# araffin/srl-zoo

Measured on AMD Instinct MI355X. Metric: images/sec (224x224x3) AE+VAE train step, higher is better.
Workload: dtype f32; 1 GPU; synthetic 224x224x3 obs, --losses autoencoder, custom_cnn, state-dim 200, bs=256 per GPU (512 frames fwd+bwd per step per GPU), Adam lr 0.005, normalised fp32 observations resident in HBM; global_batch=256, parallelism=dp1, rccl_ranks=1, devices=1

## Files before the change

### include/srlz.h

```cpp
#ifndef SRLZ_H
#define SRLZ_H

#include <stddef.h>
#include <stdint.h>

#ifdef __cplusplus
extern "C" {
#endif

typedef void* srlz_stream_t;

enum srlz_status {
  SRLZ_OK = 0,
  SRLZ_ERR_BAD_DESC = -1,
  SRLZ_ERR_WORKSPACE = -2,
  SRLZ_ERR_HIP = -3,
  SRLZ_ERR_NULL = -4
};

#define SRLZ_ABI_VERSION 104
int srlz_version(void);
const char* srlz_last_error(void);
int srlz_device_cus(void);

typedef struct {
  int n;
  int hi, wi;
  int ho, wo;
  int ksize;
  int stride;
  int pad;
  int transposed;
  int groups;
} srlz_conv64_desc;

size_t srlz_conv64_packed_floats(void);
int srlz_conv64_pack_weights(const float* w_ref, float* wpack_fwd, float* wpack_bwd,
                             const srlz_conv64_desc* d, srlz_stream_t stream);
int srlz_conv64_fwd_tiles(const srlz_conv64_desc* d);
int srlz_conv64_fwd(const float* x, const float* wpack_fwd, const float* bias, float* y, float* stats_partial,
                    const float* x_bnp, const srlz_conv64_desc* d, srlz_stream_t stream);
typedef struct {
  const float* y;
  const float* bnp;
  const float* sums;
  long long count;
  int training;
  float* dy_out;
} srlz_bn_bwd_operand;
int srlz_conv64_bwd_data(const float* dy, const float* wpack_bwd, float* dx, const srlz_bn_bwd_operand* dy_bn,
                         const srlz_conv64_desc* d, srlz_stream_t stream);
struct srlz_pool_desc_s;
int srlz_conv64_bwd_data_tiles(const srlz_conv64_desc* d);
int srlz_conv64_bwd_data_pool_sums(const float* dy, const float* wpack_bwd, float* dx, const float* pooled, const float* pool_bnp,
                                   const float* pool_y, const uint8_t* pool_argmax, const struct srlz_pool_desc_s* pd,
                                   float* bn_bwd_partial, const srlz_conv64_desc* d, srlz_stream_t stream);
int srlz_conv64_bwd_fused_supported(const srlz_conv64_desc* d);
int srlz_conv64_gather_pipe_supported(const srlz_conv64_desc* d, int backward_data);
int srlz_conv64_scatter_pipe_supported(const srlz_conv64_desc* d, int backward_data);
size_t srlz_conv64_bwd_fused_workspace(const srlz_conv64_desc* d);
int srlz_conv64_bwd_fused_bn_rows(const srlz_conv64_desc* d);
int srlz_conv64_bwd_fused_workgroups(const srlz_conv64_desc* d);
int srlz_conv64_bwd_fused(const float* x, const float* x_bnp, const float* dy, const srlz_bn_bwd_operand* dy_bn,
                          const float* wpack_bwd, float* dx, float* dw_ref, float* dbias ,
                          float* x_bn_bwd_partial , void* ws, size_t ws_bytes, const srlz_conv64_desc* d,
                          srlz_stream_t stream);
int srlz_conv64_wino_supported(const srlz_conv64_desc* d);
size_t srlz_conv64_wino_packed_floats(void);
int srlz_conv64_wino_pack_weights(const float* w_ref, float* upack_fwd, float* upack_bwd, srlz_stream_t stream);
int srlz_conv64_wino_tiles(const srlz_conv64_desc* d);
int srlz_conv64_wino_fwd(const float* x, const float* upack_fwd, const float* bias , float* y,
                         float* stats_partial , const float* x_bnp ,
                         const srlz_conv64_desc* d, srlz_stream_t stream);
int srlz_conv64_wino_bwd_data(const float* dy, const float* upack_bwd, float* dx, const srlz_conv64_desc* d, srlz_stream_t stream);
int srlz_conv64_wino_bwd_data_rows(const srlz_conv64_desc* d);
int srlz_conv64_wino_bwd_data_pool_sums(const float* dy, const float* upack_bwd, float* dx, const float* pooled, const float* pool_bnp,
                                        const float* pool_y, const uint8_t* pool_argmax, const struct srlz_pool_desc_s* pd,
                                        float* bn_bwd_partial, const srlz_conv64_desc* d, srlz_stream_t stream);
size_t srlz_conv64_wino_bwd_weight_workspace(const srlz_conv64_desc* d);
int srlz_conv64_wino_bwd_weight(const float* x, const float* dy, float* dw_ref, void* ws, size_t ws_bytes, const srlz_conv64_desc* d,
                                srlz_stream_t stream);
size_t srlz_conv64_bwd_weight_workspace(const srlz_conv64_desc* d);
int srlz_conv64_bwd_weight(const float* x, const float* dy, float* dw_ref, float* dbias, const float* x_bnp ,
                           const srlz_bn_bwd_operand* dy_bn ,
                           void* ws, size_t ws_bytes, const srlz_conv64_desc* d, srlz_stream_t stream);
int srlz_conv64_bwd_weight_plan(const srlz_conv64_desc* d, int has_x_bnp, int has_dy_bn, int out[4]);

typedef struct {
  int n, hi, wi, ho, wo;
  int cin, cout;
  int ksize, stride, pad;
  int groups;
} srlz_convn_desc;
size_t srlz_convn_packed_floats(const srlz_convn_desc* d);
int srlz_convn_pack_weights(const float* w_ref, float* wpack, const srlz_convn_desc* d, srlz_stream_t stream);
int srlz_convn_fwd_tiles(const srlz_convn_desc* d);
int srlz_convn_fwd(const float* x, const float* wpack, float* y, float* stats_partial, const float* x_bnp,
                   const srlz_convn_desc* d, srlz_stream_t stream);

typedef struct {
  int n;
  int c;
  int himg, wimg;
  int hf, wf;
  int kind;
  int groups;
} srlz_skinny_desc;

int srlz_skinny_tiles(const srlz_skinny_desc* d);
int srlz_conv1_workgroups(const srlz_skinny_desc* d);
int srlz_conv1_fwd(const float* x_nchw, const float* w_ref, float* y_nhwc, float* stats_partial,
                   const srlz_skinny_desc* d, srlz_stream_t stream);
int srlz_conv1_fwd_u8(const uint8_t* x_u8, const float* norm_lut, const float* w_ref, float* y_nhwc, float* stats_partial,
                      const srlz_skinny_desc* d, srlz_stream_t stream);
size_t srlz_skinny_bwd_weight_workspace(const srlz_skinny_desc* d);
int srlz_conv1_bwd_data(const float* dy_nhwc, const float* w_ref, float* dx_nchw, const srlz_skinny_desc* d,
                        srlz_stream_t stream);
int srlz_conv1_bwd_weight(const float* x_nchw, const float* dy_nhwc, float* dw_ref, void* ws, size_t ws_bytes,
                          const srlz_skinny_desc* d, srlz_stream_t stream);
int srlz_conv1_bwd_weight_fused(const float* x_nchw, const float* y_nhwc, const float* bnp, const uint8_t* argmax,
                                const float* dpooled, const float* sums, int training, float* dw_ref, void* ws,
                                size_t ws_bytes, const srlz_skinny_desc* d, const struct srlz_pool_desc_s* pd,
                                srlz_stream_t stream);
int srlz_conv1_bwd_weight_fused_u8(const uint8_t* x_u8, const float* norm_lut, const float* y_nhwc, const float* bnp,
                                   const uint8_t* argmax, const float* dpooled, const float* sums, int training, float* dw_ref,
                                   void* ws, size_t ws_bytes, const srlz_skinny_desc* d, const struct srlz_pool_desc_s* pd,
                                   srlz_stream_t stream);
int srlz_convT_out_fwd(const float* x_nhwc, const float* w_ref, const float* bias, float* y_nchw,
                       const float* x_bnp , const srlz_skinny_desc* d,
                       srlz_stream_t stream);
int srlz_convT_out_bwd_data(const float* dy_nchw, const float* w_ref, float* dx_nhwc, const float* x_raw,
                            const float* x_bnp, float* bn_bwd_partial, const srlz_skinny_desc* d, srlz_stream_t stream);
int srlz_convT_out_bwd_weight(const float* x_nhwc, const float* dy_nchw, float* dw_ref, float* dbias,
                              const float* x_bnp, void* ws, size_t ws_bytes, const srlz_skinny_desc* d,
                              srlz_stream_t stream);

int srlz_convT_out_bwd_fused_supported(const srlz_skinny_desc* d);
int srlz_convT_out_bwd_fused_tiles(const srlz_skinny_desc* d);
size_t srlz_convT_out_bwd_fused_workspace(const srlz_skinny_desc* d);
int srlz_convT_out_bwd_fused(const float* dy_nchw, const float* w_ref, float* dx_nhwc, const float* x_raw, const float* x_bnp,
                             float* bn_bwd_partial, float* dw_ref, float* dbias , void* ws, size_t ws_bytes,
                             const float* dy_gain_dev, float dy_gain_div, float dy_gain_coef,
                             const srlz_skinny_desc* d, srlz_stream_t stream);

int srlz_convT_out_fwd_loss_workgroups(const srlz_skinny_desc* d);
int srlz_convT_out_os_plan(const srlz_skinny_desc* d, int backward, int out[2]);
int srlz_convT_out_fwd_loss(const float* x_nhwc, const float* w_ref, const float* bias, const float* target_nchw, float* err_nchw,
                            float* dec_nchw, const float* x_bnp, double* loss_partial, const srlz_skinny_desc* d,
                            srlz_stream_t stream);
int srlz_convT_out_fwd_loss_u8(const float* x_nhwc, const float* w_ref, const float* bias, const uint8_t* target_u8,
                               const float* norm_lut, float* err_nchw, float* dec_nchw, const float* x_bnp, double* loss_partial,
                               const srlz_skinny_desc* d, srlz_stream_t stream);

int srlz_bn_finalize(const float* stats_partial, int n_partials, int groups, long long count, const float* gamma,
                     const float* beta, float eps, float momentum, int repeat, float* running_mean,
                     float* running_var, long long* num_batches_tracked ,
                     float* bnp, float* batch_stat, void* ws, size_t ws_bytes, srlz_stream_t stream);
size_t srlz_bn_finalize_chunks_workspace(int chunks, int groups);
int srlz_bn_finalize_chunks(const float* stats_partial, int tiles, int chunks, int groups, long long count, const float* gamma,
                            const float* beta, float eps, float momentum, float* running_mean, float* running_var,
                            long long* num_batches_tracked , float* bnp, void* ws, size_t ws_bytes,
                            srlz_stream_t stream);
int srlz_bn_eval_params_chunks(const float* gamma, const float* beta, const float* running_mean, const float* running_var,
                               float eps, int chunks, float* bnp, srlz_stream_t stream);
int srlz_bn_add_relu(const float* a, const float* a_bnp, const float* b, const float* b_bnp, float* out, long long pixels,
                     int chunks, int groups, srlz_stream_t stream);
int srlz_avgpool_nhwc(const float* x, float* out, int n, int hw, int c, srlz_stream_t stream);
int srlz_bn_eval_params(const float* gamma, const float* beta, const float* running_mean, const float* running_var,
                        float eps, float* bnp, srlz_stream_t stream);
int srlz_bn_replay(const float* batch_stat, float momentum, float* running_mean, float* running_var,
                   srlz_stream_t stream);
#define SRLZ_BN_REPLAY_MAX 8
typedef struct {
  const float* batch_stat;
  float* running_mean;
  float* running_var;
  long long* num_batches_tracked;
} srlz_bn_replay_item;
int srlz_bn_replay_many(const srlz_bn_replay_item* items, int n, float momentum, srlz_stream_t stream);

typedef struct srlz_pool_desc_s {
  int n, h, w;
  int hp, wp;
  int pool_pad;
  int out_nchw;
  int groups;
} srlz_pool_desc;

int srlz_bn_relu_pool_fwd(const float* y, const float* bnp, float* pooled, uint8_t* argmax,
                          const srlz_pool_desc* d, srlz_stream_t stream);
size_t srlz_bn_bwd_workspace(long long elems);
int srlz_bn_relu_pool_bwd_sums(const float* y, const float* bnp, const uint8_t* argmax, const float* dpooled,
                               const float* pooled, float* sums, float* dgamma, float* dbeta, void* ws, size_t ws_bytes,
                               const srlz_pool_desc* d, srlz_stream_t stream);
int srlz_bn_relu_pool_bwd(const float* y, const float* bnp, const uint8_t* argmax, const float* dpooled,
                          const float* pooled , float* dy, float* dgamma,
                          float* dbeta, int training, void* ws, size_t ws_bytes, const srlz_pool_desc* d,
                          srlz_stream_t stream);
int srlz_bn_relu_pool_bwd_apply(const float* y, const float* bnp, const uint8_t* argmax, const float* dpooled, const float* sums,
                                float* dy, int training, const srlz_pool_desc* d, srlz_stream_t stream);
int srlz_bn_relu_fwd(const float* y, const float* bnp, float* a, long long pixels, srlz_stream_t stream);
int srlz_bn_bwd_finalize_partials(const float* partial, int n_partials, int groups, float* sums, float* dgamma, float* dbeta,
                                  void* ws, size_t ws_bytes, srlz_stream_t stream);
int srlz_bn_relu_bwd_sums(const float* y, const float* bnp, const float* da, float* sums, float* dgamma, float* dbeta,
                          void* ws, size_t ws_bytes, long long pixels, int groups, srlz_stream_t stream);
int srlz_bn_relu_bwd(const float* y, const float* bnp, const float* da, float* dy, float* dgamma, float* dbeta,
                     int training, void* ws, size_t ws_bytes, long long pixels, int groups, srlz_stream_t stream);
int srlz_nchw_to_nhwc(const float* src, float* dst, int n, int c, int h, int w, srlz_stream_t stream);
int srlz_nhwc_to_nchw(const float* src, float* dst, int n, int c, int h, int w, srlz_stream_t stream);

int srlz_dense_supported(int M, int n, int K, int plane);
size_t srlz_dense_in_workspace(int M, int n, int K);
int srlz_dense_in_fwd(const float* x, const uint8_t* x_u8, const float* norm_lut, const float* w, const float* b, float* y, int M,
                      int n, int K, int plane, int act, void* ws, size_t ws_bytes, srlz_stream_t stream);
int srlz_dense_in_wgrad(const float* dy, const float* x, const uint8_t* x_u8, const float* norm_lut, float* dw, float* db, int M,
                        int n, int K, int plane, srlz_stream_t stream);
int srlz_dense_out_fwd(const float* z, const float* w, const float* b, float* out, int M, int n, int K, int plane,
                       srlz_stream_t stream);
int srlz_dense_out_fwd_loss_workgroups(int M, int K);
int srlz_dense_out_fwd_loss(const float* z, const float* w, const float* b, const float* target, const uint8_t* target_u8,
                            const float* norm_lut, double* partial, int M, int n, int K, int plane, int half, srlz_stream_t stream);
size_t srlz_dense_out_bwd_workspace(int M, int n, int K);
int srlz_dense_out_bwd(const float* z, const float* w, const float* b, const float* target, const uint8_t* target_u8,
                       const float* norm_lut, const float* gain, float div, float* dz, float* dw, float* db, int M, int n, int K,
                       int plane, void* ws, size_t ws_bytes, srlz_stream_t stream);
int srlz_dense_out_bwd_from(const float* dout, const float* z, const float* w, float* dz, float* dw, float* db, int M, int n, int K,
                            int plane, void* ws, size_t ws_bytes, srlz_stream_t stream);
int srlz_tanh_fwd(const float* x, float* y, int n, srlz_stream_t stream);
int srlz_tanh_bwd(const float* y, const float* dy, float* dx, int n, srlz_stream_t stream);
int srlz_add_f32(const float* a, const float* b, float* out, int n, srlz_stream_t stream);

size_t srlz_linear_workspace(int M, int N, int K);
int srlz_linear_fwd(const float* x, const float* w, const float* b, float* y, int M, int N, int K, int relu,
                    void* ws, size_t ws_bytes, srlz_stream_t stream);
int srlz_linear_fwd_res(const float* x, const float* w, const float* b, const float* res, float* y, int M, int N, int K, int relu,
                        void* ws, size_t ws_bytes, srlz_stream_t stream);
int srlz_linear_bwd_data_res(const float* dy, const float* w, const float* res, float* dx, int M, int N, int K, int Kout, void* ws,
                             size_t ws_bytes, srlz_stream_t stream);
int srlz_linear_bwd_data(const float* dy, const float* w, float* dx, int M, int N, int K, void* ws, size_t ws_bytes,
                         srlz_stream_t stream);
int srlz_linear_bwd_weight(const float* dy, const float* x, float* dw, float* db, int M, int N, int K,
                           void* ws, size_t ws_bytes, srlz_stream_t stream);
int srlz_relu_bwd_inplace(const float* y, float* dy, long long n, srlz_stream_t stream);

size_t srlz_reduce_workspace(long long n);
int srlz_sqdiff_sum(const float* a, const float* b, long long n, float* out, void* ws, size_t ws_bytes,
                    srlz_stream_t stream);
int srlz_sqdiff_sum_groups(const float* a, const float* b, long long n_per_group, int groups, float* out, void* ws,
                           size_t ws_bytes, srlz_stream_t stream);
int srlz_sqdiff_grad(const float* a, const float* b, const float* coef_dev, float coef, float* da, long long n,
                     srlz_stream_t stream);
int srlz_sqdiff_grad_groups(const float* a, const float* b, const float* coef_dev, int coef_stride, float div, float coef,
                            float* da, long long n_per_group, int groups, srlz_stream_t stream);
int srlz_pair_loss_finalize(const double* partial, int nb, long long n_per_group, int mean, float* sums, float* comb,
                            srlz_stream_t stream);
int srlz_scale_by_scalar(const float* x, const float* gain_dev, float div, float coef, float* out, long long n,
                         srlz_stream_t stream);
int srlz_sqdiff_pair_loss(const float* a, const float* b, long long n_per_group, int mean, float* sums, float* comb,
                          void* ws, size_t ws_bytes, srlz_stream_t stream);
int srlz_join2(const float* a, const float* b, float* out, long long n_each, srlz_stream_t stream);

#define SRLZ_MAX_LOSS_TERMS 15
int srlz_weighted_total(const float* const* scalars, const float* weights, int n, float* total, float* tail,
                        srlz_stream_t stream);
int srlz_weighted_total_bwd(const float* dout, const float* weights, int n, float* g, srlz_stream_t stream);
int srlz_sqdiff_mean(const float* a, const float* b, long long n, float div, float* out, void* ws, size_t ws_bytes,
                     srlz_stream_t stream);
int srlz_kl_sum(const float* mu, const float* logvar, long long n, float* out, void* ws, size_t ws_bytes,
                srlz_stream_t stream);
int srlz_kl_grad(const float* mu, const float* logvar, const float* coef_dev, float coef, float* dmu,
                 float* dlogvar, long long n, srlz_stream_t stream);
int srlz_reparam_fwd(const float* mu, const float* logvar, const float* eps, float* z, long long n,
                     srlz_stream_t stream);
int srlz_reparam_bwd(const float* dz, const float* logvar, const float* eps, float* dmu, float* dlogvar,
                     long long n, srlz_stream_t stream);
int srlz_cross_entropy(const float* logits, const int64_t* target, int B, int A, float* out, float* dlogits,
                       srlz_stream_t stream);
int srlz_prelu_fwd(const float* x, const float* slope, float* y, long long n, srlz_stream_t stream);
int srlz_prelu_bwd(const float* x, const float* slope, const float* dy, float* dx, float* dslope, long long n,
                   srlz_stream_t stream);
int srlz_triplet_fwd(const float* s, const float* p, const float* n, int B, int S, float alpha, float* out, float* hinge,
                     srlz_stream_t stream);
int srlz_triplet_bwd(const float* s, const float* p, const float* n, const float* hinge, const float* g, int B, int S,
                     float* ds, float* dp, float* dn, srlz_stream_t stream);
int srlz_cat_cols(const float* a, const float* b, float* out, int rows, int ca, int cb, srlz_stream_t stream);
int srlz_split_cols(const float* in, float* a, float* b, int rows, int ca, int cb, srlz_stream_t stream);
int srlz_sum_terms(const float* const* terms, int nterms, float* out, long long n, srlz_stream_t stream);
int srlz_concat_onehot(const float* s, const int64_t* a, float* cat, int B, int S, int A, srlz_stream_t stream);

int srlz_normalize_u8(const uint8_t* img_nhwc, float* out_ncwh, int n, int h, int w, int c, srlz_stream_t stream);
int srlz_normalize_lut(float* norm_lut, srlz_stream_t stream);
int srlz_normalize_u8_planar(const uint8_t* x_u8, const float* norm_lut, float* out, int n, int c, long long plane,
                             srlz_stream_t stream);
int srlz_copy_frames_u8(const uint8_t* src, const long long* src_index, long long src_shift, uint8_t* dst,
                        const long long* dst_index, long long dst_shift, int n, long long frame_bytes, srlz_stream_t stream);
int srlz_copy_frames_u8_strided(const uint8_t* src, const long long* src_index, long long src_shift, long long src_frame_bytes,
                                long long src_offset_bytes, uint8_t* dst, const long long* dst_index, long long dst_shift,
                                long long dst_frame_bytes, long long dst_offset_bytes, int n, long long copy_bytes, srlz_stream_t stream);
int srlz_occlude_frames_u8(const uint8_t* store, const long long* index, long long shift, const int* rects, const float* norm_lut,
                           float* out, int n, int c, int w, int h, srlz_stream_t stream);

int srlz_mask_columns(const float* x, float* y, int rows, int cols, int lo, int hi, srlz_stream_t stream);

int srlz_param_norms(const float* const* ptrs, const long long* lens, int nseg, int mode, float scale, float* norms,
                     float* out, srlz_stream_t stream);
int srlz_param_norms_grad(const float* const* ptrs, float* const* gptrs, const long long* lens, int nseg, int mode,
                          const float* norms, const float* coef_dev, float scale, srlz_stream_t stream);

int srlz_fold_grads(float* grad, float* stages, long long n, int nstage, srlz_stream_t stream);

size_t srlz_reward_prior_workspace(int S);
int srlz_reward_prior_fwd(const float* states, const float* rewards, int B, int S, float* out, double* ws, size_t ws_bytes,
                          srlz_stream_t stream);
int srlz_reward_prior_bwd(const float* states, const float* rewards, const double* ws, size_t ws_bytes, const float* g, int B, int S,
                          float* dstates, srlz_stream_t stream);
size_t srlz_episode_prior_workspace(int B, int S);
int srlz_episode_prior_fwd(const float* states, const int* others, const float* same, int B, int S, const float* w1, const float* b1,
                           const float* w2, const float* b2, const float* w3, const float* b3, float* out, void* ws, size_t ws_bytes,
                           unsigned* ticket, srlz_stream_t stream);
int srlz_episode_prior_bwd(const float* states, const int* others, const float* same, const float* g, int B, int S, const float* w1,
                           const float* w2, const float* w3, void* ws, size_t ws_bytes, float* dstates, float* dw1, float* db1,
                           float* dw2, float* db2, float* dw3, float* db3, srlz_stream_t stream);

int srlz_adam_step(float* p, const float* g, float* m, float* v, long long n, double lr, double beta1, double beta2,
                   double eps, int step, float grad_scale, srlz_stream_t stream);
int srlz_adam_step_dev(float* p, const float* g, float* m, float* v, long long n, double lr, double beta1, double beta2,
                       double eps, int* step_dev, float* bc_dev, float grad_scale, srlz_stream_t stream);

size_t srlz_comm_unique_id_bytes(void);
int srlz_comm_unique_id(void* id_out_host);
int srlz_comm_init(const void* id_host, int rank, int world);
int srlz_comm_world(void);
int srlz_comm_allreduce_f32(float* buf, long long n, srlz_stream_t stream);
int srlz_comm_destroy(void);

int srlz_mse_target_fwd(const float* pred, const float* target, int B, int S, float* loss, float* dpred_unit, srlz_stream_t stream);
int srlz_dropout_fwd(const float* x, const unsigned char* mask, float keep, float* y, int rows, int cols, srlz_stream_t stream);
int srlz_dropout_bwd(const float* dy, const unsigned char* mask, float keep, float* dx, int rows, int cols, srlz_stream_t stream);

size_t srlz_knn_workspace(int N, int Q, int D, int K);
int srlz_knn_f64(const double* db , int N, const double* queries , int Q, int D, int K, int* idx ,
                 double* dist2 , void* ws, size_t ws_bytes, srlz_stream_t stream);

size_t srlz_gtc_workspace(int N, int G, int S);
int srlz_gtc_rows_f64(const double* gt , const double* states , int N, int G, int S, double* corr ,
                      double* colstats , void* ws, size_t ws_bytes, srlz_stream_t stream);

int srlz_reward_probe_chunk_rows(int S);
int srlz_reward_probe_fit(const float* states , const int* labels , int N, int S, const int* idx ,
                          const int* idx_host , int n_steps, int B, float* params, float* m, float* v, int t0, double lr,
                          double beta1, double beta2, double eps, double* running_loss , long long* counts ,
                          double* step_loss , srlz_stream_t stream);
size_t srlz_reward_probe_eval_workspace(int n_batches, int B);
int srlz_reward_probe_eval(const float* states , const int* labels , int N, int S, const int* idx ,
                           const int* idx_host , int n_batches, int B, const float* params, double* running_loss ,
                           long long* counts , void* ws, size_t ws_bytes, unsigned* ticket, srlz_stream_t stream);

int srlz_decoded_to_bgr(const float* dec , int n, int w, int h, float* img , srlz_stream_t stream);
int srlz_decoded_to_sheet_u8(const float* dec , int n, int w, int h, int cols, int gap, int fill, int rgb,
                             unsigned char* sheet , int sheet_h, int sheet_w, srlz_stream_t stream);

size_t srlz_pca_workspace(int rows, int D);
size_t srlz_pca_transform_workspace(int M, int k, int D);
int srlz_pca_stats(const uint8_t* x_u8, const float* x_f32, const float* norm_lut, int plane, int m, int D, long long n_seen,
                   double* mean, double* var, double* bmean, double* corr, srlz_stream_t stream);
int srlz_pca_gram(const double* basis , int k, int first, const uint8_t* x_u8, const float* x_f32, const float* norm_lut,
                  int plane, int m, const double* bmean , const double* corr , int D, double* G , void* ws,
                  size_t ws_bytes, srlz_stream_t stream);
int srlz_pca_project(const double* W , const double* basis , int k, int first, const uint8_t* x_u8,
                     const float* x_f32, const float* norm_lut, int plane, int m, const double* bmean, const double* corr, int D,
                     double* out , srlz_stream_t stream);
int srlz_pca_transform(const uint8_t* x_u8, const float* x_f32, const float* norm_lut, int plane, int M, const double* mean ,
                       const double* basis , const double* S , int k, int D, float* states , void* ws,
                       size_t ws_bytes, srlz_stream_t stream);

#define SRLZ_INFER_IN 0
#define SRLZ_INFER_MID 1
#define SRLZ_INFER_LAST 2
typedef struct {
  int n;
  int c_in;
  int hi, wi;
  int kind;
  int pool_pad;
  int out_nchw;
  long long stride_n, stride_c, stride_y, stride_x;
} srlz_infer_block_desc;
int srlz_infer_block_supported(const srlz_infer_block_desc* d);
int srlz_infer_block_out_dims(const srlz_infer_block_desc* d, int* hc, int* wc, int* hp, int* wp);
int srlz_infer_tile(void);
long long srlz_infer_packed_floats(int kind, int c_in);
int srlz_infer_pack_weights(const float* w_ref, float* wpack, int kind, int c_in, srlz_stream_t stream);
int srlz_infer_block(const void* x, const float* norm_lut , const float* wpack, const float* bnp, float* out,
                     const srlz_infer_block_desc* d, srlz_stream_t stream);

int srlz_conv64_debug_program(const srlz_conv64_desc* d, int backward_data, int* out, int cap);
int srlz_linear_debug_route(int op, int M, int N, int K, int Kout, const void* a, const void* b, int has_ws, size_t ws_bytes,
                            int out[3]);
int srlz_debug_mfma_peak(float* out, int blocks, int iters, srlz_stream_t stream);
int srlz_debug_mfma_valu(float* out, int blocks, int iters, int valu_per_mfma, int kind, int split, srlz_stream_t stream);
int srlz_debug_placement(unsigned* out, int blocks, int lds_bytes, int spin, srlz_stream_t stream);

#ifdef __cplusplus
}
#endif
#endif
```

### srl-zoo_amd/csrc/skinny.hip

```cpp
#include "common.h"
#include <stdlib.h>

namespace {

constexpr int XP = 24;

template <int K, int TR = 16>
struct Geo {
  static constexpr int ROWS = 2 * (TR - 1) + K;
  static constexpr int COLS = 30 + K;
  static constexpr int KT = 3 * K * K;
  static constexpr int KS = (KT + 1) / 2;
  static constexpr int PP = ((ROWS * XP + 31) / 32) * 32 + 4;
  static constexpr int TILE_FLOATS = 3 * 2 * PP;
};

struct PoolFuse {
  const float* y;
  const uint8_t* argmax;
  const float* dpooled;
  const float* bnp;
  const float* sums;
  int HP, WP, pad, training;
  float inv_count;
};

__device__ __forceinline__ int vtile(int v, int ntiles) { return v < ntiles ? xcd_remap(v, ntiles) : ntiles; }

template <int K, int TR = 16>
__host__ __device__ constexpr int koff(int k) {
  const int kk = (k < Geo<K, TR>::KT) ? k : 0;
  const int c = kk / (K * K), ky = (kk / K) % K, kx = kk % K;
  return (c * 2 + (kx & 1)) * Geo<K, TR>::PP + ky * XP + (kx >> 1);
}

template <int K, int TR = 16>
struct ImgRegs {
  static constexpr int TOT = 3 * Geo<K, TR>::ROWS * Geo<K, TR>::COLS;
  static constexpr int PER = (TOT + 255) / 256;
  int pk[PER];
  float v[PER];
  unsigned inside;
};

template <int K, int TR = 16, int XPV = XP, int PPV = Geo<K, TR>::PP>
__device__ __forceinline__ void image_index(ImgRegs<K, TR>& r) {
  constexpr int ROWS = Geo<K, TR>::ROWS, COLS = Geo<K, TR>::COLS, TOT = ImgRegs<K, TR>::TOT;
  static_assert(6 * PPV < (1 << 17), "the LDS offset has 17 bits in pk");
#pragma unroll
  for (int j = 0; j < ImgRegs<K, TR>::PER; ++j) {
    const int idx = threadIdx.x + 256 * j;
    const int c = idx / (ROWS * COLS);
    const int rem = idx - c * (ROWS * COLS);
    const int row = rem / COLS, xl = rem - row * COLS;
    const int dst = (c * 2 + (xl & 1)) * PPV + row * XPV + (xl >> 1);
    r.pk[j] = idx < TOT ? ((dst << 14) | (c << 12) | (row << 6) | xl) : -1;
  }
}

template <int K, bool HOIST, int TR = 16>
__device__ __forceinline__ bool image_decode(const ImgRegs<K, TR>& r, int j, int& c, int& row, int& xl) {
  if (HOIST) {
    constexpr int ROWS = Geo<K, TR>::ROWS, COLS = Geo<K, TR>::COLS;
    const int idx = threadIdx.x + 256 * j;
    c = idx / (ROWS * COLS);
    const int rem = idx - c * (ROWS * COLS);
    row = rem / COLS; xl = rem - row * COLS;
    return idx < ImgRegs<K, TR>::TOT;
  }
  int pk = r.pk[j];
  asm volatile("" : "+v"(pk));
  c = (pk >> 12) & 3; row = (pk >> 6) & 63; xl = pk & 63;
  return pk >= 0;
}

template <int K, int PAD, bool HOIST = false, int TR = 16, typename PT = float>
__device__ __forceinline__ void image_request(ImgRegs<K, TR>& r, const PT* __restrict__ img, int n, int C, int cg, int H,
                                              int W, int oy0, int ox0, bool valid) {
  const int iy0 = 2 * oy0 - PAD, ix0 = 2 * ox0 - PAD;
  const int plane0 = n * C + cg * 3;
  r.inside = 0;
#pragma unroll
  for (int j = 0; j < ImgRegs<K, TR>::PER; ++j) {
    int c, row, xl;
    const bool live = image_decode<K, HOIST, TR>(r, j, c, row, xl);
    const int iy = iy0 + row, ix = ix0 + xl;
    const bool ok = valid && live && (unsigned)iy < (unsigned)H && (unsigned)ix < (unsigned)W;
    const unsigned off = ((unsigned)(plane0 + c) * (unsigned)H + (unsigned)iy) * (unsigned)W + (unsigned)ix;
    const PT raw = img[ok ? off : 0u];
    if constexpr (sizeof(PT) == 1) r.v[j] = __uint_as_float((unsigned)raw);
    else r.v[j] = raw;
    r.inside |= (ok ? 1u : 0u) << j;
  }
}

template <int K, bool HOIST = false, int TR = 16, bool U8 = false, int XPV = XP, int PPV = Geo<K, TR>::PP>
__device__ __forceinline__ void image_land(float* __restrict__ T, const ImgRegs<K, TR>& r, const float gain = 1.f,
                                           const float* __restrict__ lut = nullptr) {
  float val[ImgRegs<K, TR>::PER];
  if constexpr (U8) {
#pragma unroll
    for (int j = 0; j < ImgRegs<K, TR>::PER; ++j) {
      int c, row, xl;
      const bool live = image_decode<K, HOIST, TR>(r, j, c, row, xl);
      val[j] = lut[(live ? c : 0) * 256 + (int)__float_as_uint(r.v[j])];
    }
  } else {
#pragma unroll
    for (int j = 0; j < ImgRegs<K, TR>::PER; ++j) val[j] = r.v[j] * gain;
  }
#pragma unroll
  for (int j = 0; j < ImgRegs<K, TR>::PER; ++j) {
    int c, row, xl;
    const bool live = image_decode<K, HOIST, TR>(r, j, c, row, xl);
    int dst;
    if constexpr (HOIST) dst = (c * 2 + (xl & 1)) * PPV + row * XPV + (xl >> 1);
    else { dst = r.pk[j]; asm volatile("" : "+v"(dst)); dst >>= 14; }
    T[live ? dst : PPV - 1] = ((r.inside >> j) & 1u) ? val[j] : 0.f;
  }
}

template <int K, int PAD, bool BNBWD = false, bool MULTI = false, typename PT = float>
__global__ __launch_bounds__(256, 2) void skinny_conv_kernel(const PT* __restrict__ img,
                                                            const float* __restrict__ w_ref,
                                                            float* __restrict__ feat,
                                                            float* __restrict__ stats_partial, int N, int C, int H,
                                                            int W, int HF, int WF, int tiles_y, int tiles_x,
                                                            const float* __restrict__ y_raw,
                                                            const float* __restrict__ y_bnp, int npg,
                                                            const float* __restrict__ lut = nullptr) {
  constexpr bool U8 = sizeof(PT) == 1;
  constexpr int KT = Geo<K>::KT, KS = Geo<K>::KS;
  extern __shared__ __attribute__((aligned(16))) unsigned char smem[];
  float* T = (float*)smem;
  float* Wl = T + Geo<K>::TILE_FLOATS;
  float* red = Wl + KS * 128;
  constexpr bool PIPE = !BNBWD;
  constexpr bool HOIST = (K == 7) && !BNBWD;
  float* E = PIPE ? red + 512 : T;
  if constexpr (U8) {
    float* L = E + 4096;
    for (int i = threadIdx.x; i < 768; i += 256) L[i] = lut[i];
    lut = L;
    __syncthreads();
  }

  const int tid = threadIdx.x, lane = tid & 63, wave = tid >> 6;
  const int h = lane >> 5, l31 = lane & 31;
  const int ncg = C / 3;
  const int ntiles = N * tiles_y * tiles_x;

  auto stage_weights = [&](int cg) {
    for (int idx = tid; idx < KS * 128; idx += 256) {
      const int co = idx & 63, sh = idx >> 6;
      const int k = (sh & 1) * KS + (sh >> 1);
      float v = 0.f;
      if (k < KT) v = w_ref[((size_t)co * C + cg * 3) * (K * K) + k];
      Wl[idx] = v;
    }
  };
  if (!MULTI) stage_weights(0);

  const int tx = l31 & 15, tyl = l31 >> 4;
  const int pb0 = 2 * (wave * 4 + tyl) * XP + tx;
  const int pb1 = pb0 + 4 * XP;
  const float* wl0 = Wl + h * 64 + l31;

  ImgRegs<K> nx;
  image_index<K>(nx);
  if (PIPE && (int)blockIdx.x < ntiles) {
    const int t0 = vtile(blockIdx.x, ntiles);
    const int n = t0 / (tiles_y * tiles_x);
    const int trem = t0 - n * (tiles_y * tiles_x);
    image_request<K, PAD, false>(nx, img, n, C, 0, H, W, (trem / tiles_x) * 16, (trem % tiles_x) * 16, true);
    image_land<K, HOIST, 16, U8>(T, nx, 1.f, lut);
    if (MULTI) stage_weights(0);
  }
  for (int v = blockIdx.x; v < ntiles; v += gridDim.x) {
    const int tile = xcd_remap(v, ntiles);
    const int n = tile / (tiles_y * tiles_x);
    const int trem = tile - n * (tiles_y * tiles_x);
    const int oy0 = (trem / tiles_x) * 16, ox0 = (trem % tiles_x) * 16;
    f32x16 acc[2][2];
#pragma unroll
    for (int a = 0; a < 2; ++a)
#pragma unroll
      for (int b = 0; b < 2; ++b)
#pragma unroll
        for (int r = 0; r < 16; ++r) acc[a][b][r] = 0.f;
    const int eg = lane >> 4, eslot = lane & 15;
    f32x4 yv[BNBWD ? 16 : 1];

    for (int cg = 0; cg < ncg; ++cg) {
      __syncthreads();
      int cg2 = cg + 1;
      if (PIPE) {
        int tile2 = tile;
        if (cg2 == ncg) { cg2 = 0; tile2 = vtile(v + gridDim.x, ntiles); }
        const int n2 = tile2 / (tiles_y * tiles_x);
        const int trem2 = tile2 - n2 * (tiles_y * tiles_x);
        image_request<K, PAD, false>(nx, img, n2, C, cg2, H, W, (trem2 / tiles_x) * 16, (trem2 % tiles_x) * 16, tile2 < ntiles);
      } else {
        image_request<K, PAD, false>(nx, img, n, C, cg, H, W, oy0, ox0, true);
        image_land<K, HOIST, 16, U8>(T, nx, 1.f, lut);
        if (MULTI) stage_weights(cg);
      }
      if (BNBWD && (!MULTI || cg == 0)) {
#pragma unroll
        for (int rowq = 0; rowq < 4; ++rowq)
#pragma unroll
          for (int it = 0; it < 4; ++it) {
            const int oy = oy0 + wave * 4 + rowq, ox = ox0 + it * 4 + eg;
            const bool ok = oy < HF && ox < WF;
            yv[BNBWD ? rowq * 4 + it : 0] = *(const f32x4*)(y_raw + (ok ? ((size_t)(n * HF + oy) * WF + ox) * 64 : (size_t)0) + eslot * 4);
          }
        __builtin_amdgcn_sched_barrier(0);
      }
      if (!PIPE) __syncthreads();
#pragma unroll
      for (int s = 0; s < KS; ++s) {
        const int ko = h ? koff<K>(KS + s) : koff<K>(s);
        const float a0 = T[pb0 + ko], a1 = T[pb1 + ko];
        const float b0 = wl0[s * 128], b1 = wl0[s * 128 + 32];
        acc[0][0] = __builtin_amdgcn_mfma_f32_32x32x2f32(a0, b0, acc[0][0], 0, 0, 0);
        acc[0][1] = __builtin_amdgcn_mfma_f32_32x32x2f32(a0, b1, acc[0][1], 0, 0, 0);
        acc[1][0] = __builtin_amdgcn_mfma_f32_32x32x2f32(a1, b0, acc[1][0], 0, 0, 0);
        acc[1][1] = __builtin_amdgcn_mfma_f32_32x32x2f32(a1, b1, acc[1][1], 0, 0, 0);
      }
      if (PIPE) {
        __syncthreads();
        image_land<K, HOIST, 16, U8>(T, nx, 1.f, lut);
        if (MULTI) stage_weights(cg2);
      }
    }
    if (!PIPE) __syncthreads();
    float* Ew = E + wave * 1024;
    f32x4 s1 = {0.f, 0.f, 0.f, 0.f}, s2 = {0.f, 0.f, 0.f, 0.f};
    f32x4 bmean = s1, binv = s1, bsc = s1, bsh = s1;
    if (BNBWD) {
      const float* __restrict__ yb = y_bnp + (n / npg) * 256;
      bmean = *(const f32x4*)(yb + eslot * 4); binv = *(const f32x4*)(yb + 64 + eslot * 4);
      bsc = *(const f32x4*)(yb + 128 + eslot * 4); bsh = *(const f32x4*)(yb + 192 + eslot * 4);
      asm volatile("" : "+v"(bmean), "+v"(binv), "+v"(bsc), "+v"(bsh));
#pragma unroll
      for (int i = 0; i < 16; ++i) asm volatile("" : "+v"(yv[BNBWD ? i : 0]));
    }
#pragma unroll
    for (int rowq = 0; rowq < 4; ++rowq) {
      const int mt = rowq >> 1, half = rowq & 1;
#pragma unroll
      for (int rr = 0; rr < 8; ++rr) {
        const int il = (rr & 3) + 8 * (rr >> 2) + 4 * h;
        Ew[il * 64 + l31] = acc[mt][0][8 * half + rr];
        Ew[il * 64 + 32 + l31] = acc[mt][1][8 * half + rr];
      }
      int oy = oy0 + wave * 4 + rowq;
      if (BNBWD) asm volatile("" : "+v"(oy));
#pragma unroll
      for (int it = 0; it < 4; ++it) {
        const int pl = it * 4 + eg, ox = ox0 + pl;
        const f32x4 v = *(const f32x4*)(Ew + pl * 64 + eslot * 4);
        if (oy < HF && ox < WF) {
          *(f32x4*)(feat + ((size_t)(n * HF + oy) * WF + ox) * 64 + eslot * 4) = v;
          if (BNBWD) {
            const f32x4 yy = yv[BNBWD ? rowq * 4 + it : 0];
#pragma unroll
            for (int e = 0; e < 4; ++e)
              if (yy[e] * bsc[e] + bsh[e] > 0.f) { s1[e] += v[e]; s2[e] += v[e] * ((yy[e] - bmean[e]) * binv[e]); }
          } else {
#pragma unroll
            for (int e = 0; e < 4; ++e) { s1[e] += v[e]; s2[e] += v[e] * v[e]; }
          }
        }
      }
    }
    if (stats_partial) {
#pragma unroll
      for (int e = 0; e < 4; ++e) {
        s1[e] += __shfl_xor(s1[e], 16, 64); s1[e] += __shfl_xor(s1[e], 32, 64);
        s2[e] += __shfl_xor(s2[e], 16, 64); s2[e] += __shfl_xor(s2[e], 32, 64);
      }
      if (eg == 0) {
        *(f32x4*)(red + wave * 128 + eslot * 4) = s1;
        *(f32x4*)(red + wave * 128 + 64 + eslot * 4) = s2;
      }
      __syncthreads();
      if (tid < 128) stats_partial[(size_t)tile * 128 + tid] = red[tid] + red[128 + tid] + red[256 + tid] + red[384 + tid];
    }
  }
}

constexpr int DG_NF = 11;
constexpr int DG_NPROD = 147;
constexpr int DG_TP = 149;

__global__ __launch_bounds__(256, 2) void conv1_dgrad_kernel(const float* __restrict__ dy, const float* __restrict__ w_ref,
                                                            float* __restrict__ dx, int N, int C, int H, int W, int HF,
                                                            int WF, int tiles_y, int tiles_x) {
  extern __shared__ __attribute__((aligned(16))) unsigned char smem[];
  float* Tt = (float*)smem;
  const int tid = threadIdx.x, lane = tid & 63, wave = tid >> 6;
  const int li = lane & 15, kq = lane >> 4;
  const int cg = blockIdx.y;
  const int ntiles = N * tiles_y * tiles_x;

  f32x4 breg[3][4];
#pragma unroll
  for (int j = 0; j < 3; ++j) {
    const int ncol = (wave + 4 * j) * 16 + li;
    const bool valid = (wave + 4 * j) < 10 && ncol < DG_NPROD;
    const int co = valid ? ncol / 49 : 0, tap = valid ? ncol % 49 : 0;
#pragma unroll
    for (int c = 0; c < 4; ++c)
#pragma unroll
      for (int r = 0; r < 4; ++r)
        breg[j][c][r] = valid ? w_ref[((size_t)(16 * c + 4 * kq + r) * C + cg * 3 + co) * 49 + tap] : 0.f;
  }

  for (int tile = blockIdx.x; tile < ntiles; tile += gridDim.x) {
    const int n = tile / (tiles_y * tiles_x);
    const int trem = tile - n * (tiles_y * tiles_x);
    const int ty = trem / tiles_x, tx = trem % tiles_x;
    const int fy0 = 8 * ty - 1, fx0 = 8 * tx - 1;
    __syncthreads();
    auto load_a = [&](int mtile, f32x4 (&a)[4]) {
      const int p = mtile * 16 + li;
      const int ia = p / DG_NF, ib = p - ia * DG_NF;
      const int fy = fy0 + ia, fx = fx0 + ib;
      const bool ok = mtile < 8 && p < DG_NF * DG_NF && fy >= 0 && fy < HF && fx >= 0 && fx < WF;
      const float* src = dy + ((size_t)(n * HF + (ok ? fy : 0)) * WF + (ok ? fx : 0)) * 64 + 4 * kq;
#pragma unroll
      for (int c = 0; c < 4; ++c) a[c] = ok ? *(const f32x4*)(src + 16 * c) : f32x4{0.f, 0.f, 0.f, 0.f};
    };
    f32x4 a[4], an[4];
    load_a(0, a);
#pragma unroll 1
    for (int mtile = 0; mtile < 8; ++mtile) {
      load_a(mtile + 1, an);
#pragma unroll
      for (int j = 0; j < 3; ++j) {
        if (wave + 4 * j < 10) {
          f32x4 acc = {0.f, 0.f, 0.f, 0.f};
#pragma unroll
          for (int c = 0; c < 4; ++c)
#pragma unroll
            for (int r = 0; r < 4; ++r) acc = __builtin_amdgcn_mfma_f32_16x16x4f32(a[c][r], breg[j][c][r], acc, 0, 0, 0);
          const int ncol = (wave + 4 * j) * 16 + li;
          if (ncol < DG_NPROD) {
#pragma unroll
            for (int r = 0; r < 4; ++r) Tt[(mtile * 16 + kq * 4 + r) * DG_TP + ncol] = acc[r];
          }
        }
      }
#pragma unroll
      for (int c = 0; c < 4; ++c) a[c] = an[c];
    }
    __syncthreads();
    const int oxl = tid & 15, oyl = tid >> 4;
    const int iy = 16 * ty + oyl, ix = 16 * tx + oxl;
    const int py = (oyl + 1) & 1, px = (oxl + 1) & 1;
    const int ay = (oyl + 3 - py) / 2 + 1, ax = (oxl + 3 - px) / 2 + 1;
#pragma unroll
    for (int co = 0; co < 3; ++co) {
      float v = 0.f;
#pragma unroll
      for (int dyk = 0; dyk < 4; ++dyk) {
        const int ky = py + 2 * dyk;
        if (ky > 6) continue;
#pragma unroll
        for (int dxk = 0; dxk < 4; ++dxk) {
          const int kx = px + 2 * dxk;
          if (kx > 6) continue;
          v += Tt[((ay - dyk) * DG_NF + (ax - dxk)) * DG_TP + co * 49 + ky * 7 + kx];
        }
      }
      if (iy < H && ix < W) dx[((size_t)(n * C + cg * 3 + co) * H + iy) * W + ix] = v;
    }
  }
}

constexpr int WG7_XP = 23, WG7_PP = 861;
__constant__ unsigned char TAP7[160] = {
      0,   1,   2,   4,   5,   7,   8,  11,  12,  13,  14,  15,  18,  19,  20,  21,
     25,  27,  28,  32,  33,  35,  42,  58,  59,  89,  96, 108, 124, 138, 255, 255,
     10,  22,  26,  29,  30,  31,  34,  36,  37,  38,  41,  43,  44,  45,  48,  50,
     51,  53,  57,  60,  64,  67,  72,  74,  75,  88, 101, 107, 114, 137, 255, 255,
      9,  23,  39,  49,  54,  55,  56,  61,  62,  63,  68,  69,  70,  71,  76,  77,
     78,  79,  84,  85,  86,  91,  92,  93, 115, 123, 130, 131, 140, 255, 255, 255,
      6,  17,  47,  52,  66,  73,  80,  82,  83,  87,  90,  94,  97,  99, 102, 103,
    104, 106, 109, 110, 111, 113, 116, 117, 118, 121, 125, 141, 144, 255, 255, 255,
      3,  16,  24,  40,  46,  65,  81,  95,  98, 100, 105, 112, 119, 120, 122, 126,
    127, 128, 129, 132, 133, 134, 135, 136, 139, 142, 143, 145, 146, 255, 255, 255};

template <int K, int PAD, bool FUSED = false, typename PT = float>
__global__ __launch_bounds__(256, 2) void skinny_wgrad_kernel(const PT* __restrict__ img,
                                                             const float* __restrict__ feat,
                                                             float* __restrict__ partial, int N, int C, int H, int W,
                                                             int HF, int WF, int tiles_y, int tiles_x,
                                                             const float* __restrict__ feat_bnp, const PoolFuse pf, int npg,
                                                             const float* __restrict__ lut = nullptr) {
  constexpr bool U8 = sizeof(PT) == 1;
  constexpr int KT = Geo<K>::KT;
  constexpr int NT = (KT + 31) / 32;
  extern __shared__ __attribute__((aligned(16))) unsigned char smem[];
  float* T = (float*)smem;
  float* F = T + Geo<K>::TILE_FLOATS;
  if constexpr (U8) {
    float* L = F + 128 * 64;
    for (int i = threadIdx.x; i < 768; i += 256) L[i] = lut[i];
    lut = L;
  }
  constexpr int RPS = FUSED ? 4 : 8, NSTAGE = 16 / RPS;

  const int tid = threadIdx.x, lane = tid & 63, wave = tid >> 6;
  const int h = lane >> 5, l31 = lane & 31;
  const int mt = wave & 1, sub = wave >> 1;
  const int cg = blockIdx.y;
  const int ntiles = N * tiles_y * tiles_x;
  const int tpi = tiles_y * tiles_x;

  constexpr bool DEALT = (K == 7);
  constexpr int WXP = DEALT ? WG7_XP : XP, WPP = DEALT ? WG7_PP : Geo<K>::PP;
  static_assert(6 * WPP <= Geo<K>::TILE_FLOATS && Geo<K>::ROWS * WXP <= WPP - 1, "window does not fit its planes");
  int kb[NT];
#pragma unroll
  for (int j = 0; j < NT; ++j) {
    const int k = j * 32 + l31;
    int kk = (k < KT) ? k : 0;
    if constexpr (DEALT) { kk = TAP7[k]; if (kk == 255) kk = TAP7[j * 32]; }
    const int c = kk / (K * K), ky = (kk / K) % K, kx = kk % K;
    kb[j] = (c * 2 + (kx & 1)) * WPP + ky * WXP + (kx >> 1) + h;
  }
  f32x16 acc[NT];
#pragma unroll
  for (int j = 0; j < NT; ++j)
#pragma unroll
    for (int r = 0; r < 16; ++r) acc[j][r] = 0.f;
  const float* tb[NT];
#pragma unroll
  for (int j = 0; j < NT; ++j) tb[j] = T + kb[j];
  const float* fcol = F + h * 64 + mt * 32 + l31;

  const int slot = tid & 15, prow = tid >> 4;
  f32x4 sc4 = {1.f, 1.f, 1.f, 1.f}, sh4 = {0.f, 0.f, 0.f, 0.f};
  f32x4 fc0 = {0.f, 0.f, 0.f, 0.f}, fc1 = {0.f, 0.f, 0.f, 0.f};
  int cur_grp = -1;
  f32x4 pv[RPS];
  unsigned pmask = 0;
  f32x4 dpv[FUSED ? 2 : 1][2];
  uint32_t am[FUSED ? 2 : 1][2];
  unsigned wmask = 0;
  bool all_win = false;
  const int brow = (tid >> 4) >> 3, bcol = (tid >> 4) & 7;
  auto f_request = [&](int tile_, int half_) {
    const int n_ = tile_ / tpi;
    const int trem_ = tile_ - n_ * tpi;
    const int oy0_ = (trem_ / tiles_x) * 16, ox0_ = (trem_ % tiles_x) * 16;
    const bool live = tile_ < ntiles;
    const float* __restrict__ fsrc = FUSED ? pf.y : feat;
    pmask = 0;
    if constexpr (FUSED) {
      all_win = live && ((oy0_ + RPS * half_) >> 1) + RPS / 2 < pf.HP && (ox0_ >> 1) + 8 < pf.WP;
      const int oyb = oy0_ + RPS * half_ + 2 * brow, oxb = ox0_ + 2 * bcol;
#pragma unroll
      for (int i = 0; i < 2; ++i)
#pragma unroll
        for (int j = 0; j < 2; ++j) {
          const int oy = oyb + i, ox = oxb + j;
          const bool ok = live && oy < HF && ox < WF;
          pv[2 * i + j] = *(const f32x4*)(fsrc + (ok ? ((size_t)(n_ * HF + oy) * WF + ox) * 64 : (size_t)0) + slot * 4);
          pmask |= (ok ? 1u : 0u) << (2 * i + j);
        }
      wmask = 0;
#pragma unroll
      for (int wy = 0; wy < 2; ++wy)
#pragma unroll
        for (int wx = 0; wx < 2; ++wx) {
          const int py = (oyb >> 1) + wy, px = (oxb >> 1) + wx;
          const bool ok = live && py < pf.HP && px < pf.WP;
          const size_t pp = (ok ? ((size_t)(n_ * pf.HP + py) * pf.WP + px) * 64 : (size_t)0) + slot * 4;
          am[wy][wx] = *(const uint32_t*)(pf.argmax + pp);
          dpv[wy][wx] = *(const f32x4*)(pf.dpooled + pp);
          wmask |= (ok ? 1u : 0u) << (2 * wy + wx);
        }
    } else {
#pragma unroll
      for (int j = 0; j < RPS; ++j) {
        const int oy = oy0_ + RPS * half_ + j, ox = ox0_ + prow;
        const bool ok = live && oy < HF && ox < WF;
        pv[j] = *(const f32x4*)(fsrc + (ok ? ((size_t)(n_ * HF + oy) * WF + ox) * 64 : (size_t)0) + slot * 4);
        pmask |= (ok ? 1u : 0u) << j;
      }
    }
  };
  auto f_resolve = [&]() {
    if constexpr (FUSED) {
      uint32_t a[2][2];
#pragma unroll
      for (int wy = 0; wy < 2; ++wy)
#pragma unroll
        for (int wx = 0; wx < 2; ++wx) a[wy][wx] = am[wy][wx];
      if (!all_win) {
#pragma unroll
        for (int wy = 0; wy < 2; ++wy)
#pragma unroll
          for (int wx = 0; wx < 2; ++wx) a[wy][wx] = ((wmask >> (2 * wy + wx)) & 1u) ? am[wy][wx] : 0xffffffffu;
      }
#pragma unroll
      for (int i = 0; i < 2; ++i)
#pragma unroll
        for (int j = 0; j < 2; ++j) {
          f32x4 dz = {0.f, 0.f, 0.f, 0.f};
#pragma unroll
          for (int wy = 0; wy <= i; ++wy)
#pragma unroll
            for (int wx = 0; wx <= j; ++wx) {
              const uint32_t code = (uint32_t)((i - 2 * wy + 1) * 3 + (j - 2 * wx + 1));
#pragma unroll
              for (int e = 0; e < 4; ++e)
                if (((a[wy][wx] >> (8 * e)) & 0xffu) == code) dz[e] += dpv[wy][wx][e];
            }
          const f32x4 yy = pv[2 * i + j];
          f32x4 o;
#pragma unroll
          for (int e = 0; e < 4; ++e) {
            const float z = yy[e] * sc4[e] + sh4[e];
            const float d = z > 0.f ? dz[e] : 0.f;
            o[e] = sc4[e] * d - (fc0[e] + fc1[e] * yy[e]);
          }
          if (!((pmask >> (2 * i + j)) & 1u)) o = f32x4{0.f, 0.f, 0.f, 0.f};
          *(f32x4*)(F + (16 * (2 * brow + i) + 2 * bcol + j) * 64 + slot * 4) = o;
        }
    } else {
      if (K == 4 && feat_bnp) {
#pragma unroll
        for (int j = 0; j < RPS; ++j) {
          const bool ok = (pmask >> j) & 1u;
#pragma unroll
          for (int e = 0; e < 4; ++e) { const float z = pv[j][e] * sc4[e] + sh4[e]; pv[j][e] = (ok && z > 0.f) ? z : 0.f; }
        }
      }
      else {
#pragma unroll
        for (int j = 0; j < RPS; ++j)
          if (!((pmask >> j) & 1u)) pv[j] = f32x4{0.f, 0.f, 0.f, 0.f};
      }
#pragma unroll
      for (int j = 0; j < RPS; ++j) *(f32x4*)(F + (16 * j + prow) * 64 + slot * 4) = pv[j];
    }
  };
  ImgRegs<K> ir;
  image_index<K, 16, WXP, WPP>(ir);
  auto i_request = [&](int tile_) {
    const int n_ = tile_ / tpi;
    const int trem_ = tile_ - n_ * tpi;
    image_request<K, PAD, K == 4>(ir, img, n_, C, cg, H, W, (trem_ / tiles_x) * 16, (trem_ % tiles_x) * 16, tile_ < ntiles);
  };
  if ((int)blockIdx.x < ntiles) { f_request(vtile(blockIdx.x, ntiles), 0); i_request(vtile(blockIdx.x, ntiles)); }
  for (int v = blockIdx.x; v < ntiles; v += gridDim.x) {
    const int tile = xcd_remap(v, ntiles);
    const int n = tile / tpi;
    const int grp = n / npg;
    if (grp != cur_grp) {
      cur_grp = grp;
      if constexpr (FUSED) {
        const float* __restrict__ pbnp = pf.bnp + grp * 256;
        const float* __restrict__ psums = pf.sums + grp * 128;
        const f32x4 mean = *(const f32x4*)(pbnp + slot * 4), invstd = *(const f32x4*)(pbnp + 64 + slot * 4);
        sc4 = *(const f32x4*)(pbnp + 128 + slot * 4); sh4 = *(const f32x4*)(pbnp + 192 + slot * 4);
        f32x4 m1 = *(const f32x4*)(psums + slot * 4), m2 = *(const f32x4*)(psums + 64 + slot * 4);
        if (!pf.training) m1 = m2 = f32x4{0.f, 0.f, 0.f, 0.f};
#pragma unroll
        for (int e = 0; e < 4; ++e) {
          fc1[e] = sc4[e] * invstd[e] * m2[e] * pf.inv_count;
          fc0[e] = sc4[e] * m1[e] * pf.inv_count - fc1[e] * mean[e];
        }
      } else if (K == 4 && feat_bnp) {
        sc4 = *(const f32x4*)(feat_bnp + grp * 256 + 128 + slot * 4);
        sh4 = *(const f32x4*)(feat_bnp + grp * 256 + 192 + slot * 4);
      }
    }
#pragma unroll 1
    for (int half = 0; half < NSTAGE; ++half) {
      __syncthreads();
      if (half == 0) image_land<K, K == 4, 16, U8, WXP, WPP>(T, ir, 1.f, lut);
      f_resolve();
      __syncthreads();
      if (half + 1 < NSTAGE) f_request(tile, half + 1);
      else { f_request(vtile(v + gridDim.x, ntiles), 0); i_request(vtile(v + gridDim.x, ntiles)); }
      const int subu = __builtin_amdgcn_readfirstlane(sub);
#pragma unroll 2
      for (int blk = 0; blk < RPS; ++blk) {
        const int lrow = (RPS / 2) * subu + (blk >> 1), tx0 = 8 * (blk & 1);
        const float* fa = fcol + (lrow * 16 + tx0) * 64;
        const int boff = 2 * (RPS * half + lrow) * WXP + tx0;
        float a[4], b[NT][4];
#pragma unroll
        for (int i = 0; i < 4; ++i) a[i] = fa[2 * i * 64];
#pragma unroll
        for (int j = 0; j < NT; ++j)
#pragma unroll
          for (int i = 0; i < 4; ++i) b[j][i] = tb[j][boff + 2 * i];
#pragma unroll
        for (int i = 0; i < 4; ++i)
#pragma unroll
          for (int j = 0; j < NT; ++j) acc[j] = __builtin_amdgcn_mfma_f32_32x32x2f32(a[i], b[j][i], acc[j], 0, 0, 0);
      }
    }
  }
  float* out = partial + (((size_t)cg * gridDim.x + blockIdx.x) * 2 + sub) * (64 * NT * 32);
#pragma unroll
  for (int j = 0; j < NT; ++j) {
    int col = j * 32 + l31;
    if constexpr (DEALT) col = TAP7[col];
    if (col == 255) continue;
#pragma unroll
    for (int r = 0; r < 16; ++r) {
      const int row = mt * 32 + (r & 3) + 8 * (r >> 2) + 4 * h;
      out[row * (NT * 32) + col] = acc[j][r];
    }
  }
}

constexpr int WRED_OUTS = 64, WRED_PARTS = 16;
__global__ __launch_bounds__(1024) void skinny_wgrad_reduce(const float* __restrict__ partial, int nwg, int C, int KK, int KT,
                                                           int NTW, float* __restrict__ dw_ref) {
  const int o = threadIdx.x & (WRED_OUTS - 1), part = threadIdx.x / WRED_OUTS;
  const int id = blockIdx.x * WRED_OUTS + o;
  const int ncg = C / 3;
  const bool live = id < ncg * 64 * KT;
  int cg = 0, ch = 0, k = 0;
  double s0 = 0.0, s1 = 0.0, s2 = 0.0, s3 = 0.0;
  if (live) {
    cg = id / (64 * KT);
    const int rem = id - cg * 64 * KT;
    ch = rem / KT; k = rem - ch * KT;
    const float* base = partial + (size_t)cg * nwg * (64 * NTW) + ch * NTW + k;
    const int per = (nwg + WRED_PARTS - 1) / WRED_PARTS;
    const int w0 = part * per, w1 = (w0 + per < nwg) ? w0 + per : nwg;
    int w = w0;
    for (; w + 3 < w1; w += 4) {
      s0 += (double)base[(size_t)w * (64 * NTW)];
      s1 += (double)base[(size_t)(w + 1) * (64 * NTW)];
      s2 += (double)base[(size_t)(w + 2) * (64 * NTW)];
      s3 += (double)base[(size_t)(w + 3) * (64 * NTW)];
    }
    for (; w < w1; ++w) s0 += (double)base[(size_t)w * (64 * NTW)];
  }
  __shared__ double sm[WRED_PARTS][WRED_OUTS];
  sm[part][o] = (s0 + s1) + (s2 + s3);
  __syncthreads();
  if (part == 0 && live) {
    double t = 0.0;
#pragma unroll
    for (int q = 0; q < WRED_PARTS; ++q) t += sm[q][o];
    dw_ref[((size_t)ch * C + cg * 3) * KK + k] = (float)t;
  }
}

__global__ __launch_bounds__(256) void nchw_chan_sum_partial(const float* __restrict__ x, int C, int HW, double* __restrict__ partial,
                                                            int N) {
  const int n = blockIdx.x / C, c = blockIdx.x % C;
  const float* plane = x + (size_t)blockIdx.x * HW;
  float s = 0.f;
  const int hw4 = HW >> 2;
  for (int i = threadIdx.x; i < hw4; i += 256) {
    const f32x4 v = *(const f32x4*)(plane + i * 4);
    s += (v[0] + v[1]) + (v[2] + v[3]);
  }
  for (int i = hw4 * 4 + threadIdx.x; i < HW; i += 256) s += plane[i];
  const double d = block_sum_pairs_d((double)s);
  if (threadIdx.x == 0) partial[(size_t)c * N + n] = d;
}
__global__ void nchw_chan_sum_final(const double* __restrict__ partial, int N, float* __restrict__ out) {
  const int c = blockIdx.x;
  double s = 0.0;
  for (int i = threadIdx.x; i < N; i += 64) s += partial[(size_t)c * N + i];
  s = wave_sum_d(s);
  if (threadIdx.x == 0) out[c] = (float)s;
}

static int check_skinny(const srlz_skinny_desc* d) {
  SRLZ_REQUIRE(d != nullptr, SRLZ_ERR_NULL, "skinny: null descriptor");
  SRLZ_REQUIRE((long long)d->n * d->c * d->himg * d->wimg < (1LL << 31), SRLZ_ERR_BAD_DESC,
               "skinny: image tensor of %lld elements (the window staging keeps 32-bit element offsets)",
               (long long)d->n * d->c * d->himg * d->wimg);
  SRLZ_REQUIRE(d->n > 0 && d->c > 0 && d->c % 3 == 0 && d->c <= 9, SRLZ_ERR_BAD_DESC, "skinny: C must be 3, 6 or 9 (got %d)", d->c);
  SRLZ_REQUIRE(d->groups >= 0 && (d->groups <= 1 || d->n % d->groups == 0), SRLZ_ERR_BAD_DESC,
               "skinny: n = %d is not a multiple of groups = %d", d->n, d->groups);
  if (d->kind == 0) {
    SRLZ_REQUIRE(d->hf == (d->himg + 6 - 7) / 2 + 1 && d->wf == (d->wimg + 6 - 7) / 2 + 1, SRLZ_ERR_BAD_DESC,
                 "conv1: feature map %dx%d inconsistent with image %dx%d", d->hf, d->wf, d->himg, d->wimg);
  } else if (d->kind == 1) {
    SRLZ_REQUIRE(d->himg == (d->hf - 1) * 2 + 4 && d->wimg == (d->wf - 1) * 2 + 4, SRLZ_ERR_BAD_DESC,
                 "convT_out: image %dx%d inconsistent with feature map %dx%d", d->himg, d->wimg, d->hf, d->wf);
  } else {
    SRLZ_REQUIRE(false, SRLZ_ERR_BAD_DESC, "skinny: unknown kind %d", d->kind);
  }
  return 0;
}

template <int K>
static size_t conv_lds(bool pipe) { return (size_t)(Geo<K>::TILE_FLOATS + Geo<K>::KS * 128 + 512 + (pipe ? 4096 : 0)) * 4; }

static int images_per_group(const srlz_skinny_desc* d) { return d->n / (d->groups > 1 ? d->groups : 1); }

static int persistent_grid(int ntiles) {
  const int g = 2 * srlz_device_cus();
  return g > ntiles ? ntiles : g;
}

template <int K, int PAD, typename PT = float>
static int launch_conv(const PT* img, const float* w, float* feat, float* stats, const srlz_skinny_desc* d, hipStream_t st,
                       const float* y_raw = nullptr, const float* y_bnp = nullptr, const float* lut = nullptr) {
  const int ty = (d->hf + 15) / 16, tx = (d->wf + 15) / 16;
  const int ntiles = d->n * ty * tx;
  const bool multi = d->c > 3;
  const dim3 grid(persistent_grid(ntiles)), block(256);
#define SRLZ_CONV_LAUNCH(BN, MU, PIPED)                                                                                   \
  do {                                                                                                                    \
    const size_t lds = conv_lds<K>(PIPED) + (sizeof(PT) == 1 ? 768 * 4 : 0);                                              \
    SRLZ_MAX_LDS((skinny_conv_kernel<K, PAD, BN, MU, PT>), lds);                                                          \
    SRLZ_LAUNCH((skinny_conv_kernel<K, PAD, BN, MU, PT>), grid, block, lds, st, img, w, feat, stats, d->n, d->c,          \
                d->himg, d->wimg, d->hf, d->wf, ty, tx, y_raw, y_bnp, images_per_group(d), lut);                          \
  } while (0)
  bool launched = false;
  if constexpr (K == 4 && sizeof(PT) == 4) if (y_raw) {
    if (multi) SRLZ_CONV_LAUNCH(true, true, false); else SRLZ_CONV_LAUNCH(true, false, false);
    launched = true;
  }
  if (!launched) {
    if (multi) SRLZ_CONV_LAUNCH(false, true, true); else SRLZ_CONV_LAUNCH(false, false, true);
  }
#undef SRLZ_CONV_LAUNCH
  return 0;
}

template <int K>
static size_t wgrad_ws(const srlz_skinny_desc* d) {
  constexpr int NT = (Geo<K>::KT + 31) / 32;
  const int ty = (d->hf + 15) / 16, tx = (d->wf + 15) / 16;
  const int g = persistent_grid(d->n * ty * tx);
  return (size_t)(d->c / 3) * g * 2 * 64 * NT * 32 * sizeof(float) + (size_t)d->n * d->c * sizeof(double);
}

template <int K, int PAD, typename PT = float>
static int launch_wgrad(const PT* img, const float* feat, float* dw, void* ws, size_t ws_bytes, const srlz_skinny_desc* d,
                        hipStream_t st, const float* feat_bnp = nullptr, const PoolFuse* pfuse = nullptr, const float* lut = nullptr) {
  constexpr int NT = (Geo<K>::KT + 31) / 32;
  const int ty = (d->hf + 15) / 16, tx = (d->wf + 15) / 16;
  const int ntiles = d->n * ty * tx;
  const int g = persistent_grid(ntiles);
  SRLZ_REQUIRE(ws_bytes >= wgrad_ws<K>(d), SRLZ_ERR_WORKSPACE, "skinny wgrad: workspace too small (%zu)", ws_bytes);
  SRLZ_REQUIRE(K == 4 || feat_bnp == nullptr, SRLZ_ERR_BAD_DESC, "skinny wgrad: a fused forward operand exists for the 4x4 layer only");
  const size_t lds = (size_t)(Geo<K>::TILE_FLOATS + 128 * 64) * 4 + (sizeof(PT) == 1 ? 768 * 4 : 0);
  float* partial = (float*)ws;
  PoolFuse pf = {};
  if (pfuse) pf = *pfuse;
  bool launched = false;
  if constexpr (K == 7) if (pf.y) {
    SRLZ_LAUNCH((skinny_wgrad_kernel<K, PAD, true, PT>), dim3(g, d->c / 3), dim3(256), lds, st, img, feat, partial, d->n, d->c, d->himg,
                d->wimg, d->hf, d->wf, ty, tx, feat_bnp, pf, images_per_group(d), lut);
    launched = true;
  }
  if (!launched)
    SRLZ_LAUNCH((skinny_wgrad_kernel<K, PAD, false, PT>), dim3(g, d->c / 3), dim3(256), lds, st, img, feat, partial, d->n, d->c, d->himg,
                d->wimg, d->hf, d->wf, ty, tx, feat_bnp, pf, images_per_group(d), lut);
  const int total = (d->c / 3) * 64 * Geo<K>::KT;
  SRLZ_LAUNCH(skinny_wgrad_reduce, dim3((total + WRED_OUTS - 1) / WRED_OUTS), dim3(1024), 0, st, partial, 2 * g, d->c, K * K, Geo<K>::KT,
              NT * 32, dw);
  return 0;
}

}

extern "C" int srlz_skinny_tiles(const srlz_skinny_desc* d) {
  if (check_skinny(d)) return -1;
  return d->n * ((d->hf + 15) / 16) * ((d->wf + 15) / 16);
}

extern "C" int srlz_conv1_workgroups(const srlz_skinny_desc* d) {
  if (check_skinny(d) || d->kind != 0) return -1;
  return persistent_grid(d->n * ((d->hf + 15) / 16) * ((d->wf + 15) / 16));
}

extern "C" int srlz_conv1_fwd(const float* x_nchw, const float* w_ref, float* y_nhwc, float* stats_partial,
                              const srlz_skinny_desc* d, srlz_stream_t stream) {
  if (int rc = check_skinny(d)) return rc;
  SRLZ_REQUIRE(d->kind == 0, SRLZ_ERR_BAD_DESC, "conv1_fwd: descriptor kind must be 0");
  SRLZ_REQUIRE(x_nchw && w_ref && y_nhwc, SRLZ_ERR_NULL, "conv1_fwd: null pointer");
  return launch_conv<7, 3>(x_nchw, w_ref, y_nhwc, stats_partial, d, as_stream(stream));
}

extern "C" int srlz_conv1_fwd_u8(const uint8_t* x_u8, const float* norm_lut, const float* w_ref, float* y_nhwc,
                                 float* stats_partial, const srlz_skinny_desc* d, srlz_stream_t stream) {
  if (int rc = check_skinny(d)) return rc;
  SRLZ_REQUIRE(d->kind == 0, SRLZ_ERR_BAD_DESC, "conv1_fwd_u8: descriptor kind must be 0");
  SRLZ_REQUIRE(x_u8 && norm_lut && w_ref && y_nhwc, SRLZ_ERR_NULL, "conv1_fwd_u8: null pointer");
  return launch_conv<7, 3, uint8_t>(x_u8, w_ref, y_nhwc, stats_partial, d, as_stream(stream), nullptr, nullptr, norm_lut);
}

extern "C" size_t srlz_skinny_bwd_weight_workspace(const srlz_skinny_desc* d) {
  if (check_skinny(d)) return 0;
  return d->kind == 0 ? wgrad_ws<7>(d) : wgrad_ws<4>(d);
}

extern "C" int srlz_conv1_bwd_data(const float* dy_nhwc, const float* w_ref, float* dx_nchw, const srlz_skinny_desc* d,
                                   srlz_stream_t stream) {
  if (int rc = check_skinny(d)) return rc;
  SRLZ_REQUIRE(d->kind == 0, SRLZ_ERR_BAD_DESC, "conv1_bwd_data: descriptor kind must be 0");
  SRLZ_REQUIRE(dy_nhwc && w_ref && dx_nchw, SRLZ_ERR_NULL, "conv1_bwd_data: null pointer");
  const int ty = (d->himg + 15) / 16, tx = (d->wimg + 15) / 16;
  const int ntiles = d->n * ty * tx;
  const size_t lds = (size_t)128 * DG_TP * sizeof(float);
  SRLZ_MAX_LDS(conv1_dgrad_kernel, lds);
  SRLZ_LAUNCH(conv1_dgrad_kernel, dim3(persistent_grid(ntiles), d->c / 3), dim3(256), lds, as_stream(stream), dy_nhwc, w_ref, dx_nchw, d->n,
              d->c, d->himg, d->wimg, d->hf, d->wf, ty, tx);
  return 0;
}

extern "C" int srlz_conv1_bwd_weight(const float* x_nchw, const float* dy_nhwc, float* dw_ref, void* ws, size_t ws_bytes,
                                     const srlz_skinny_desc* d, srlz_stream_t stream) {
  if (int rc = check_skinny(d)) return rc;
  SRLZ_REQUIRE(d->kind == 0, SRLZ_ERR_BAD_DESC, "conv1_bwd_weight: descriptor kind must be 0");
  SRLZ_REQUIRE(x_nchw && dy_nhwc && dw_ref && ws, SRLZ_ERR_NULL, "conv1_bwd_weight: null pointer");
  return launch_wgrad<7, 3>(x_nchw, dy_nhwc, dw_ref, ws, ws_bytes, d, as_stream(stream));
}

template <typename PT>
static int conv1_bwd_weight_fused(const PT* x_nchw, const float* lut, const float* y_nhwc, const float* bnp, const uint8_t* argmax,
                                  const float* dpooled, const float* sums, int training, float* dw_ref, void* ws,
                                  size_t ws_bytes, const srlz_skinny_desc* d, const srlz_pool_desc* pd,
                                  srlz_stream_t stream) {
  if (int rc = check_skinny(d)) return rc;
  SRLZ_REQUIRE(d->kind == 0 && pd, SRLZ_ERR_BAD_DESC, "conv1_bwd_weight_fused: descriptor kind must be 0");
  SRLZ_REQUIRE(x_nchw && y_nhwc && bnp && argmax && dpooled && sums && dw_ref && ws, SRLZ_ERR_NULL,
               "conv1_bwd_weight_fused: null pointer");
  SRLZ_REQUIRE(pd->n == d->n && pd->h == d->hf && pd->w == d->wf && !pd->out_nchw && pd->pool_pad == 1 &&
               (pd->groups > 1 ? pd->groups : 1) == (d->groups > 1 ? d->groups : 1), SRLZ_ERR_BAD_DESC,
               "conv1_bwd_weight_fused: pooling descriptor does not match conv1's output");
  PoolFuse pf;
  pf.y = y_nhwc; pf.argmax = argmax; pf.dpooled = dpooled; pf.bnp = bnp; pf.sums = sums;
  pf.HP = pd->hp; pf.WP = pd->wp; pf.pad = pd->pool_pad; pf.training = training;
  pf.inv_count = 1.0f / (float)((double)images_per_group(d) * d->hf * d->wf);
  return launch_wgrad<7, 3, PT>(x_nchw, y_nhwc, dw_ref, ws, ws_bytes, d, as_stream(stream), nullptr, &pf, lut);
}

extern "C" int srlz_conv1_bwd_weight_fused(const float* x_nchw, const float* y_nhwc, const float* bnp, const uint8_t* argmax,
                                           const float* dpooled, const float* sums, int training, float* dw_ref, void* ws,
                                           size_t ws_bytes, const srlz_skinny_desc* d, const srlz_pool_desc* pd,
                                           srlz_stream_t stream) {
  return conv1_bwd_weight_fused<float>(x_nchw, nullptr, y_nhwc, bnp, argmax, dpooled, sums, training, dw_ref, ws, ws_bytes, d, pd,
                                       stream);
}

extern "C" int srlz_conv1_bwd_weight_fused_u8(const uint8_t* x_u8, const float* norm_lut, const float* y_nhwc, const float* bnp,
                                              const uint8_t* argmax, const float* dpooled, const float* sums, int training,
                                              float* dw_ref, void* ws, size_t ws_bytes, const srlz_skinny_desc* d,
                                              const srlz_pool_desc* pd, srlz_stream_t stream) {
  SRLZ_REQUIRE(norm_lut, SRLZ_ERR_NULL, "conv1_bwd_weight_fused_u8: null normalisation table");
  return conv1_bwd_weight_fused<uint8_t>(x_u8, norm_lut, y_nhwc, bnp, argmax, dpooled, sums, training, dw_ref, ws, ws_bytes, d, pd,
                                         stream);
}

extern "C" int srlz_convT_out_bwd_data(const float* dy_nchw, const float* w_ref, float* dx_nhwc, const float* x_raw,
                                       const float* x_bnp, float* bn_bwd_partial, const srlz_skinny_desc* d,
                                       srlz_stream_t stream) {
  if (int rc = check_skinny(d)) return rc;
  SRLZ_REQUIRE(d->kind == 1, SRLZ_ERR_BAD_DESC, "convT_out_bwd_data: descriptor kind must be 1");
  SRLZ_REQUIRE(dy_nchw && w_ref && dx_nhwc, SRLZ_ERR_NULL, "convT_out_bwd_data: null pointer");
  SRLZ_REQUIRE((x_raw != nullptr) == (x_bnp != nullptr) && (x_raw != nullptr) == (bn_bwd_partial != nullptr), SRLZ_ERR_NULL,
               "convT_out_bwd_data: x_raw, x_bnp and bn_bwd_partial go together");
  return launch_conv<4, 0>(dy_nchw, w_ref, dx_nhwc, bn_bwd_partial, d, as_stream(stream), x_raw, x_bnp);
}

extern "C" int srlz_convT_out_bwd_weight(const float* x_nhwc, const float* dy_nchw, float* dw_ref, float* dbias,
                                         const float* x_bnp, void* ws, size_t ws_bytes, const srlz_skinny_desc* d,
                                         srlz_stream_t stream) {
  if (int rc = check_skinny(d)) return rc;
  SRLZ_REQUIRE(d->kind == 1, SRLZ_ERR_BAD_DESC, "convT_out_bwd_weight: descriptor kind must be 1");
  SRLZ_REQUIRE(x_nhwc && dy_nchw && dw_ref && ws, SRLZ_ERR_NULL, "convT_out_bwd_weight: null pointer");
  if (int rc = launch_wgrad<4, 0>(dy_nchw, x_nhwc, dw_ref, ws, ws_bytes, d, as_stream(stream), x_bnp)) return rc;
  if (dbias) {
    double* part = (double*)((char*)ws + wgrad_ws<4>(d) - (size_t)d->n * d->c * sizeof(double));
    SRLZ_REQUIRE((((uintptr_t)part) & 7) == 0 && ((d->himg * d->wimg) & 3) == 0, SRLZ_ERR_BAD_DESC,
                 "convT_out_bwd_weight: unaligned workspace / image plane");
    SRLZ_LAUNCH(nchw_chan_sum_partial, dim3(d->n * d->c), dim3(256), 0, as_stream(stream), dy_nchw, d->c, d->himg * d->wimg, part, d->n);
    SRLZ_LAUNCH(nchw_chan_sum_final, dim3(d->c), dim3(64), 0, as_stream(stream), part, d->n, dbias);
  }
  return 0;
}
```

### srl-zoo_amd/srlz/_cabi.py

```python
import ctypes
import os
from ctypes import c_int, c_longlong, c_float, c_double, c_void_p, c_size_t, c_char_p, POINTER, Structure

_HERE = os.path.dirname(os.path.abspath(__file__))
LIB_PATH = os.path.join(_HERE, "libsrlz_hip.so")


ABI_VERSION = 104


class SrlzError(RuntimeError):
    pass


class Conv64Desc(Structure):
    _fields_ = [("n", c_int), ("hi", c_int), ("wi", c_int), ("ho", c_int), ("wo", c_int), ("ksize", c_int),
                ("stride", c_int), ("pad", c_int), ("transposed", c_int), ("groups", c_int)]


class SkinnyDesc(Structure):
    _fields_ = [("n", c_int), ("c", c_int), ("himg", c_int), ("wimg", c_int), ("hf", c_int), ("wf", c_int),
                ("kind", c_int), ("groups", c_int)]


class PoolDesc(Structure):
    _fields_ = [("n", c_int), ("h", c_int), ("w", c_int), ("hp", c_int), ("wp", c_int), ("pool_pad", c_int),
                ("out_nchw", c_int), ("groups", c_int)]


class ConvNDesc(Structure):
    _fields_ = [("n", c_int), ("hi", c_int), ("wi", c_int), ("ho", c_int), ("wo", c_int), ("cin", c_int), ("cout", c_int),
                ("ksize", c_int), ("stride", c_int), ("pad", c_int), ("groups", c_int)]

    def __init__(self, n, hi, wi, ho, wo, cin, cout, ksize, stride, pad, groups=1):
        super(ConvNDesc, self).__init__(n, hi, wi, ho, wo, cin, cout, ksize, stride, pad, groups)


class BnReplayItem(Structure):
    _fields_ = [("batch_stat", c_void_p), ("running_mean", c_void_p), ("running_var", c_void_p), ("num_batches_tracked", c_void_p)]


class BnBwdOperand(Structure):
    _fields_ = [("y", c_void_p), ("bnp", c_void_p), ("sums", c_void_p), ("count", c_longlong), ("training", c_int),
                ("dy_out", c_void_p)]


class InferBlockDesc(Structure):
    _fields_ = [("n", c_int), ("c_in", c_int), ("hi", c_int), ("wi", c_int), ("kind", c_int), ("pool_pad", c_int),
                ("out_nchw", c_int), ("stride_n", c_longlong), ("stride_c", c_longlong), ("stride_y", c_longlong),
                ("stride_x", c_longlong)]


INFER_IN, INFER_MID, INFER_LAST = 0, 1, 2

P = c_void_p
_BO = POINTER(BnBwdOperand)
_C64 = POINTER(Conv64Desc)
_SK = POINTER(SkinnyDesc)
_PD = POINTER(PoolDesc)
_CN = POINTER(ConvNDesc)
_IB = POINTER(InferBlockDesc)

_PROTOS = {
    "srlz_version": (c_int, []),
    "srlz_last_error": (c_char_p, []),
    "srlz_device_cus": (c_int, []),
    "srlz_conv64_packed_floats": (c_size_t, []),
    "srlz_conv64_pack_weights": (c_int, [P, P, P, _C64, P]),
    "srlz_conv64_fwd_tiles": (c_int, [_C64]),
    "srlz_conv64_fwd": (c_int, [P, P, P, P, P, P, _C64, P]),
    "srlz_conv64_bwd_data": (c_int, [P, P, P, _BO, _C64, P]),
    "srlz_conv64_bwd_weight_workspace": (c_size_t, [_C64]),
    "srlz_conv64_bwd_fused_supported": (c_int, [_C64]),
    "srlz_conv64_gather_pipe_supported": (c_int, [_C64, c_int]),
    "srlz_conv64_scatter_pipe_supported": (c_int, [_C64, c_int]),
    "srlz_conv64_bwd_fused_workspace": (c_size_t, [_C64]),
    "srlz_conv64_bwd_fused": (c_int, [P, P, P, _BO, P, P, P, P, P, P, c_size_t, _C64, P]),
    "srlz_conv64_bwd_fused_bn_rows": (c_int, [_C64]),
    "srlz_conv64_wino_supported": (c_int, [_C64]),
    "srlz_conv64_wino_packed_floats": (c_size_t, []),
    "srlz_conv64_wino_pack_weights": (c_int, [P, P, P, P]),
    "srlz_conv64_wino_tiles": (c_int, [_C64]),
    "srlz_conv64_wino_fwd": (c_int, [P, P, P, P, P, P, _C64, P]),
    "srlz_conv64_wino_bwd_data": (c_int, [P, P, P, _C64, P]),
    "srlz_conv64_wino_bwd_weight_workspace": (c_size_t, [_C64]),
    "srlz_conv64_wino_bwd_weight": (c_int, [P, P, P, P, c_size_t, _C64, P]),
    "srlz_conv64_wino_bwd_data_rows": (c_int, [_C64]),
    "srlz_conv64_wino_bwd_data_pool_sums": (c_int, [P, P, P, P, P, P, P, _PD, P, _C64, P]),
    "srlz_conv64_bwd_weight": (c_int, [P, P, P, P, P, _BO, P, c_size_t, _C64, P]),
    "srlz_conv64_bwd_weight_plan": (c_int, [_C64, c_int, c_int, POINTER(c_int)]),
    "srlz_conv64_bwd_fused_workgroups": (c_int, [_C64]),
    "srlz_conv1_workgroups": (c_int, [_SK]),
    "srlz_convT_out_os_plan": (c_int, [_SK, c_int, POINTER(c_int)]),
    "srlz_conv64_debug_program": (c_int, [_C64, c_int, POINTER(c_int), c_int]),
    "srlz_linear_debug_route": (c_int, [c_int, c_int, c_int, c_int, c_int, P, P, c_int, c_size_t, POINTER(c_int)]),
    "srlz_debug_placement": (c_int, [P, c_int, c_int, c_int, P]),
    "srlz_debug_mfma_peak": (c_int, [P, c_int, c_int, P]),
    "srlz_debug_mfma_valu": (c_int, [P, c_int, c_int, c_int, c_int, c_int, P]),
    "srlz_convn_packed_floats": (c_size_t, [_CN]),
    "srlz_convn_pack_weights": (c_int, [P, P, _CN, P]),
    "srlz_convn_fwd_tiles": (c_int, [_CN]),
    "srlz_convn_fwd": (c_int, [P, P, P, P, P, _CN, P]),
    "srlz_bn_finalize_chunks_workspace": (c_size_t, [c_int, c_int]),
    "srlz_bn_finalize_chunks": (c_int, [P, c_int, c_int, c_int, c_longlong, P, P, c_float, c_float, P, P, P, P, P, c_size_t, P]),
    "srlz_bn_eval_params_chunks": (c_int, [P, P, P, P, c_float, c_int, P, P]),
    "srlz_bn_add_relu": (c_int, [P, P, P, P, P, c_longlong, c_int, c_int, P]),
    "srlz_avgpool_nhwc": (c_int, [P, P, c_int, c_int, c_int, P]),
    "srlz_prelu_fwd": (c_int, [P, P, P, c_longlong, P]),
    "srlz_prelu_bwd": (c_int, [P, P, P, P, P, c_longlong, P]),
    "srlz_triplet_fwd": (c_int, [P, P, P, c_int, c_int, c_float, P, P, P]),
    "srlz_triplet_bwd": (c_int, [P, P, P, P, P, c_int, c_int, P, P, P, P]),
    "srlz_skinny_tiles": (c_int, [_SK]),
    "srlz_conv64_bwd_data_tiles": (c_int, [_C64]),
    "srlz_conv64_bwd_data_pool_sums": (c_int, [P, P, P, P, P, P, P, _PD, P, _C64, P]),
    "srlz_conv1_fwd": (c_int, [P, P, P, P, _SK, P]),
    "srlz_conv1_fwd_u8": (c_int, [P, P, P, P, P, _SK, P]),
    "srlz_conv1_bwd_weight_fused_u8": (c_int, [P, P, P, P, P, P, P, c_int, P, P, c_size_t, _SK, _PD, P]),
    "srlz_convT_out_fwd_loss_u8": (c_int, [P, P, P, P, P, P, P, P, P, _SK, P]),
    "srlz_normalize_lut": (c_int, [P, P]),
    "srlz_normalize_u8_planar": (c_int, [P, P, P, c_int, c_int, c_longlong, P]),
    "srlz_copy_frames_u8": (c_int, [P, P, c_longlong, P, P, c_longlong, c_int, c_longlong, P]),
    "srlz_copy_frames_u8_strided": (c_int, [P, P, c_longlong, c_longlong, c_longlong, P, P, c_longlong, c_longlong, c_longlong, c_int,
                                            c_longlong, P]),
    "srlz_occlude_frames_u8": (c_int, [P, P, c_longlong, P, P, P, c_int, c_int, c_int, c_int, P]),
    "srlz_skinny_bwd_weight_workspace": (c_size_t, [_SK]),
    "srlz_conv1_bwd_weight": (c_int, [P, P, P, P, c_size_t, _SK, P]),
    "srlz_conv1_bwd_data": (c_int, [P, P, P, _SK, P]),
    "srlz_conv1_bwd_weight_fused": (c_int, [P, P, P, P, P, P, c_int, P, P, c_size_t, _SK, _PD, P]),
    "srlz_bn_relu_pool_bwd_sums": (c_int, [P, P, P, P, P, P, P, P, P, c_size_t, _PD, P]),
    "srlz_convT_out_fwd": (c_int, [P, P, P, P, P, _SK, P]),
    "srlz_convT_out_bwd_data": (c_int, [P, P, P, P, P, P, _SK, P]),
    "srlz_bn_bwd_finalize_partials": (c_int, [P, c_int, c_int, P, P, P, P, c_size_t, P]),
    "srlz_convT_out_bwd_weight": (c_int, [P, P, P, P, P, P, c_size_t, _SK, P]),
    "srlz_convT_out_bwd_fused_supported": (c_int, [_SK]),
    "srlz_convT_out_bwd_fused_tiles": (c_int, [_SK]),
    "srlz_convT_out_bwd_fused_workspace": (c_size_t, [_SK]),
    "srlz_convT_out_bwd_fused": (c_int, [P, P, P, P, P, P, P, P, P, c_size_t, P, c_float, c_float, _SK, P]),
    "srlz_convT_out_fwd_loss_workgroups": (c_int, [_SK]),
    "srlz_convT_out_fwd_loss": (c_int, [P, P, P, P, P, P, P, P, _SK, P]),
    "srlz_pair_loss_finalize": (c_int, [P, c_int, c_longlong, c_int, P, P, P]),
    "srlz_scale_by_scalar": (c_int, [P, P, c_float, c_float, P, c_longlong, P]),
    "srlz_bn_finalize": (c_int, [P, c_int, c_int, c_longlong, P, P, c_float, c_float, c_int, P, P, P, P, P, P, c_size_t, P]),
    "srlz_bn_eval_params": (c_int, [P, P, P, P, c_float, P, P]),
    "srlz_bn_replay": (c_int, [P, c_float, P, P, P]),
    "srlz_bn_replay_many": (c_int, [POINTER(BnReplayItem), c_int, c_float, P]),
    "srlz_bn_relu_pool_fwd": (c_int, [P, P, P, P, _PD, P]),
    "srlz_bn_bwd_workspace": (c_size_t, [c_longlong]),
    "srlz_bn_relu_pool_bwd": (c_int, [P, P, P, P, P, P, P, P, c_int, P, c_size_t, _PD, P]),
    "srlz_bn_relu_pool_bwd_apply": (c_int, [P, P, P, P, P, P, c_int, _PD, P]),
    "srlz_bn_relu_fwd": (c_int, [P, P, P, c_longlong, P]),
    "srlz_bn_relu_bwd_sums": (c_int, [P, P, P, P, P, P, P, c_size_t, c_longlong, c_int, P]),
    "srlz_bn_relu_bwd": (c_int, [P, P, P, P, P, P, c_int, P, c_size_t, c_longlong, c_int, P]),
    "srlz_nchw_to_nhwc": (c_int, [P, P, c_int, c_int, c_int, c_int, P]),
    "srlz_nhwc_to_nchw": (c_int, [P, P, c_int, c_int, c_int, c_int, P]),
    "srlz_dense_supported": (c_int, [c_int, c_int, c_int, c_int]),
    "srlz_dense_in_workspace": (c_size_t, [c_int, c_int, c_int]),
    "srlz_dense_in_fwd": (c_int, [P, P, P, P, P, P, c_int, c_int, c_int, c_int, c_int, P, c_size_t, P]),
    "srlz_dense_in_wgrad": (c_int, [P, P, P, P, P, P, c_int, c_int, c_int, c_int, P]),
    "srlz_dense_out_fwd": (c_int, [P, P, P, P, c_int, c_int, c_int, c_int, P]),
    "srlz_dense_out_fwd_loss_workgroups": (c_int, [c_int, c_int]),
    "srlz_dense_out_fwd_loss": (c_int, [P, P, P, P, P, P, P, c_int, c_int, c_int, c_int, c_int, P]),
    "srlz_dense_out_bwd_workspace": (c_size_t, [c_int, c_int, c_int]),
    "srlz_dense_out_bwd": (c_int, [P, P, P, P, P, P, P, c_float, P, P, P, c_int, c_int, c_int, c_int, P, c_size_t, P]),
    "srlz_dense_out_bwd_from": (c_int, [P, P, P, P, P, P, c_int, c_int, c_int, c_int, P, c_size_t, P]),
    "srlz_tanh_fwd": (c_int, [P, P, c_int, P]),
    "srlz_tanh_bwd": (c_int, [P, P, P, c_int, P]),
    "srlz_add_f32": (c_int, [P, P, P, c_int, P]),
    "srlz_linear_workspace": (c_size_t, [c_int, c_int, c_int]),
    "srlz_linear_fwd": (c_int, [P, P, P, P, c_int, c_int, c_int, c_int, P, c_size_t, P]),
    "srlz_linear_bwd_data": (c_int, [P, P, P, c_int, c_int, c_int, P, c_size_t, P]),
    "srlz_linear_fwd_res": (c_int, [P, P, P, P, P, c_int, c_int, c_int, c_int, P, c_size_t, P]),
    "srlz_linear_bwd_data_res": (c_int, [P, P, P, P, c_int, c_int, c_int, c_int, P, c_size_t, P]),
    "srlz_cat_cols": (c_int, [P, P, P, c_int, c_int, c_int, P]),
    "srlz_split_cols": (c_int, [P, P, P, c_int, c_int, c_int, P]),
    "srlz_sum_terms": (c_int, [P, c_int, P, c_longlong, P]),
    "srlz_sqdiff_mean": (c_int, [P, P, c_longlong, c_float, P, P, c_size_t, P]),
    "srlz_linear_bwd_weight": (c_int, [P, P, P, P, c_int, c_int, c_int, P, c_size_t, P]),
    "srlz_relu_bwd_inplace": (c_int, [P, P, c_longlong, P]),
    "srlz_reduce_workspace": (c_size_t, [c_longlong]),
    "srlz_sqdiff_sum": (c_int, [P, P, c_longlong, P, P, c_size_t, P]),
    "srlz_sqdiff_grad": (c_int, [P, P, P, c_float, P, c_longlong, P]),
    "srlz_sqdiff_sum_groups": (c_int, [P, P, c_longlong, c_int, P, P, c_size_t, P]),
    "srlz_sqdiff_grad_groups": (c_int, [P, P, P, c_int, c_float, c_float, P, c_longlong, c_int, P]),
    "srlz_sqdiff_pair_loss": (c_int, [P, P, c_longlong, c_int, P, P, P, c_size_t, P]),
    "srlz_join2": (c_int, [P, P, P, c_longlong, P]),
    "srlz_weighted_total": (c_int, [P, P, c_int, P, P, P]),
    "srlz_weighted_total_bwd": (c_int, [P, P, c_int, P, P]),
    "srlz_kl_sum": (c_int, [P, P, c_longlong, P, P, c_size_t, P]),
    "srlz_kl_grad": (c_int, [P, P, P, c_float, P, P, c_longlong, P]),
    "srlz_reparam_fwd": (c_int, [P, P, P, P, c_longlong, P]),
    "srlz_reparam_bwd": (c_int, [P, P, P, P, P, c_longlong, P]),
    "srlz_cross_entropy": (c_int, [P, P, c_int, c_int, P, P, P]),
    "srlz_reward_prior_workspace": (c_size_t, [c_int]),
    "srlz_reward_prior_fwd": (c_int, [P, P, c_int, c_int, P, P, c_size_t, P]),
    "srlz_reward_prior_bwd": (c_int, [P, P, P, c_size_t, P, c_int, c_int, P, P]),
    "srlz_episode_prior_workspace": (c_size_t, [c_int, c_int]),
    "srlz_episode_prior_fwd": (c_int, [P, P, P, c_int, c_int, P, P, P, P, P, P, P, P, c_size_t, P, P]),
    "srlz_episode_prior_bwd": (c_int, [P, P, P, P, c_int, c_int, P, P, P, P, c_size_t, P, P, P, P, P, P, P, P]),
    "srlz_knn_workspace": (c_size_t, [c_int, c_int, c_int, c_int]),
    "srlz_knn_f64": (c_int, [P, c_int, P, c_int, c_int, c_int, P, P, P, c_size_t, P]),
    "srlz_gtc_workspace": (c_size_t, [c_int, c_int, c_int]),
    "srlz_gtc_rows_f64": (c_int, [P, P, c_int, c_int, c_int, P, P, P, c_size_t, P]),
    "srlz_reward_probe_chunk_rows": (c_int, [c_int]),
    "srlz_reward_probe_fit": (c_int, [P, P, c_int, c_int, P, P, c_int, c_int, P, P, P, c_int, c_double, c_double, c_double, c_double, P,
                                      P, P, P]),
    "srlz_reward_probe_eval_workspace": (c_size_t, [c_int, c_int]),
    "srlz_reward_probe_eval": (c_int, [P, P, c_int, c_int, P, P, c_int, c_int, P, P, P, P, c_size_t, P, P]),
    "srlz_decoded_to_bgr": (c_int, [P, c_int, c_int, c_int, P, P]),
    "srlz_decoded_to_sheet_u8": (c_int, [P, c_int, c_int, c_int, c_int, c_int, c_int, c_int, P, c_int, c_int, P]),
    "srlz_pca_workspace": (c_size_t, [c_int, c_int]),
    "srlz_pca_transform_workspace": (c_size_t, [c_int, c_int, c_int]),
    "srlz_pca_stats": (c_int, [P, P, P, c_int, c_int, c_int, c_longlong, P, P, P, P, P]),
    "srlz_pca_gram": (c_int, [P, c_int, c_int, P, P, P, c_int, c_int, P, P, c_int, P, P, c_size_t, P]),
    "srlz_pca_project": (c_int, [P, P, c_int, c_int, P, P, P, c_int, c_int, P, P, c_int, P, P]),
    "srlz_pca_transform": (c_int, [P, P, P, c_int, c_int, P, P, P, c_int, c_int, P, P, c_size_t, P]),
    "srlz_mse_target_fwd": (c_int, [P, P, c_int, c_int, P, P, P]),
    "srlz_dropout_fwd": (c_int, [P, P, c_float, P, c_int, c_int, P]),
    "srlz_dropout_bwd": (c_int, [P, P, c_float, P, c_int, c_int, P]),
    "srlz_concat_onehot": (c_int, [P, P, P, c_int, c_int, c_int, P]),
    "srlz_normalize_u8": (c_int, [P, P, c_int, c_int, c_int, c_int, P]),
    "srlz_mask_columns": (c_int, [P, P, c_int, c_int, c_int, c_int, P]),
    "srlz_param_norms": (c_int, [P, P, c_int, c_int, c_float, P, P, P]),
    "srlz_param_norms_grad": (c_int, [P, P, P, c_int, c_int, P, P, c_float, P]),
    "srlz_fold_grads": (c_int, [P, P, c_longlong, c_int, P]),
    "srlz_comm_unique_id_bytes": (c_size_t, []),
    "srlz_comm_unique_id": (c_int, [P]),
    "srlz_comm_init": (c_int, [P, c_int, c_int]),
    "srlz_comm_world": (c_int, []),
    "srlz_comm_allreduce_f32": (c_int, [P, c_longlong, P]),
    "srlz_comm_destroy": (c_int, []),
    "srlz_adam_step": (c_int, [P, P, P, P, c_longlong, c_double, c_double, c_double, c_double, c_int, c_float, P]),
    "srlz_adam_step_dev": (c_int, [P, P, P, P, c_longlong, c_double, c_double, c_double, c_double, P, P, c_float, P]),
    "srlz_infer_block_supported": (c_int, [_IB]),
    "srlz_infer_block_out_dims": (c_int, [_IB, POINTER(c_int), POINTER(c_int), POINTER(c_int), POINTER(c_int)]),
    "srlz_infer_tile": (c_int, []),
    "srlz_infer_packed_floats": (c_longlong, [c_int, c_int]),
    "srlz_infer_pack_weights": (c_int, [P, P, c_int, c_int, P]),
    "srlz_infer_block": (c_int, [P, P, P, P, P, _IB, P]),
}

_NOT_STATUS = {"srlz_version", "srlz_device_cus", "srlz_conv64_fwd_tiles", "srlz_skinny_tiles", "srlz_convn_fwd_tiles",
               "srlz_convT_out_bwd_fused_tiles", "srlz_convT_out_fwd_loss_workgroups", "srlz_conv64_bwd_fused_supported", "srlz_conv64_gather_pipe_supported",
               "srlz_conv64_scatter_pipe_supported",
               "srlz_convT_out_bwd_fused_supported",
               "srlz_conv64_bwd_data_tiles", "srlz_conv64_bwd_fused_bn_rows", "srlz_conv64_wino_supported", "srlz_conv64_wino_packed_floats",
               "srlz_conv64_wino_tiles", "srlz_conv64_wino_bwd_data_rows",
               "srlz_conv64_debug_program", "srlz_comm_world", "srlz_dense_supported",
               "srlz_dense_out_fwd_loss_workgroups", "srlz_reward_probe_chunk_rows", "srlz_infer_block_supported",
               "srlz_infer_tile", "srlz_conv64_bwd_fused_workgroups", "srlz_conv1_workgroups"}

EXPORTED = sorted(_PROTOS.keys())


def _load():
    if not os.path.exists(LIB_PATH):
        raise SrlzError(
            "libsrlz_hip.so not found at %s — build it with `python -c 'import __graft_entry__ as g; g.build()'` "
            "(or `make -C srl-zoo_amd/csrc`). There is no CPU fallback for the srl-zoo_amd hot path." % LIB_PATH)
    lib = ctypes.CDLL(LIB_PATH)
    for name, (res, args) in _PROTOS.items():
        fn = getattr(lib, name)
        fn.restype = res
        fn.argtypes = args
    got = lib.srlz_version()
    if got != ABI_VERSION:
        raise SrlzError("libsrlz_hip.so at %s reports ABI version %d, these bindings are written for %d (include/srlz.h "
                        "SRLZ_ABI_VERSION): rebuild with `make -C srl-zoo_amd/csrc`" % (LIB_PATH, got, ABI_VERSION))
    return lib


_lib = _load()


def error_text():
    return _lib.srlz_last_error().decode("utf-8", "replace")


_DEBUG_SYNC = bool(os.environ.get("SRLZ_SYNC"))


def _wrap(name):
    fn = getattr(_lib, name)
    if _PROTOS[name][0] is c_int and name not in _NOT_STATUS:
        def call(*a):
            rc = fn(*a)
            if rc != 0:
                raise SrlzError("%s failed (%d): %s" % (name, rc, error_text()))
            if _DEBUG_SYNC:
                import torch
                torch.cuda.synchronize()
            return rc
        call.__name__ = name
        return call
    return fn


for _n in _PROTOS:
    globals()[_n[len("srlz_"):]] = _wrap(_n)


def ptr(t):
    if t is None:
        return None
    return c_void_p(t.data_ptr())


def stream():
    import torch
    return c_void_p(torch.cuda.current_stream().cuda_stream)
```

Baseline: 44920 images/s.

## Stage conv1 image tiles and feature stores through raw buffer loads

Adds a buffer-resource path for the 7x7 stem convolution forward and its fused weight-gradient kernel. Image windows are fetched with raw buffer loads using precomputed per-lane byte offsets, and out-of-range lanes use an out-of-bounds offset that the hardware drops instead of branching. Forward feature stores go through buffer stores, with a full-tile fast path and zeroing of the accumulators folded into the first MFMA step. The aim is to cut address arithmetic and bounds-check work in the staging loops, at the cost of more registers per lane for the offsets and some extra template complexity. The older generic path stays reachable through new debug entry points.

Result: faster. 45410 images/s (median of 6 runs) (+1.1%).

```diff
diff --git a/include/srlz.h b/include/srlz.h
--- a/include/srlz.h
+++ b/include/srlz.h
@@ -109,6 +109,7 @@
 
 int srlz_skinny_tiles(const srlz_skinny_desc* d);
 int srlz_conv1_workgroups(const srlz_skinny_desc* d);
+int srlz_conv1_buffer_staging_supported(const srlz_skinny_desc* d);
 int srlz_conv1_fwd(const float* x_nchw, const float* w_ref, float* y_nhwc, float* stats_partial,
                    const srlz_skinny_desc* d, srlz_stream_t stream);
 int srlz_conv1_fwd_u8(const uint8_t* x_u8, const float* norm_lut, const float* w_ref, float* y_nhwc, float* stats_partial,
@@ -400,6 +401,18 @@
 int srlz_debug_mfma_peak(float* out, int blocks, int iters, srlz_stream_t stream);
 int srlz_debug_mfma_valu(float* out, int blocks, int iters, int valu_per_mfma, int kind, int split, srlz_stream_t stream);
 int srlz_debug_placement(unsigned* out, int blocks, int lds_bytes, int spin, srlz_stream_t stream);
+int srlz_debug_conv1_fwd_generic(const float* x_nchw, const float* w_ref, float* y_nhwc, float* stats_partial,
+                                 const srlz_skinny_desc* d, srlz_stream_t stream);
+int srlz_debug_conv1_fwd_u8_generic(const uint8_t* x_u8, const float* norm_lut, const float* w_ref, float* y_nhwc,
+                                    float* stats_partial, const srlz_skinny_desc* d, srlz_stream_t stream);
+int srlz_debug_conv1_bwd_weight_fused_generic(const float* x_nchw, const float* y_nhwc, const float* bnp, const uint8_t* argmax,
+                                              const float* dpooled, const float* sums, int training, float* dw_ref, void* ws,
+                                              size_t ws_bytes, const srlz_skinny_desc* d, const struct srlz_pool_desc_s* pd,
+                                              srlz_stream_t stream);
+int srlz_debug_conv1_bwd_weight_fused_u8_generic(const uint8_t* x_u8, const float* norm_lut, const float* y_nhwc, const float* bnp,
+                                                 const uint8_t* argmax, const float* dpooled, const float* sums, int training,
+                                                 float* dw_ref, void* ws, size_t ws_bytes, const srlz_skinny_desc* d,
+                                                 const struct srlz_pool_desc_s* pd, srlz_stream_t stream);
 
 #ifdef __cplusplus
 }
diff --git a/srl-zoo_amd/csrc/skinny.hip b/srl-zoo_amd/csrc/skinny.hip
--- a/srl-zoo_amd/csrc/skinny.hip
+++ b/srl-zoo_amd/csrc/skinny.hip
@@ -1,5 +1,6 @@
 #include "common.h"
 #include <stdlib.h>
+#include <type_traits>
 
 namespace {
 
@@ -39,6 +40,7 @@
   static constexpr int TOT = 3 * Geo<K, TR>::ROWS * Geo<K, TR>::COLS;
   static constexpr int PER = (TOT + 255) / 256;
   int pk[PER];
+  unsigned voff[PER];
   float v[PER];
   unsigned inside;
 };
@@ -120,8 +122,105 @@
   }
 }
 
-template <int K, int PAD, bool BNBWD = false, bool MULTI = false, typename PT = float>
-__global__ __launch_bounds__(256, 2) void skinny_conv_kernel(const PT* __restrict__ img,
+constexpr unsigned IMG_DROP = 0xFFFFFF00u;
+
+template <typename T> struct BufStaged {};
+template <typename T> struct Pixel { using type = T; static constexpr bool buf = false; };
+template <typename T> struct Pixel<BufStaged<T>> { using type = T; static constexpr bool buf = true; };
+
+template <int K, typename PT, bool VOFF, int TR = 16, int XPV = XP, int PPV = Geo<K, TR>::PP>
+__device__ __forceinline__ void image_index_buf(ImgRegs<K, TR>& r, int H, int W) {
+  constexpr int ROWS = Geo<K, TR>::ROWS, COLS = Geo<K, TR>::COLS, TOT = ImgRegs<K, TR>::TOT;
+  static_assert(6 * PPV < (1 << 17) && ROWS < 64 && COLS < 64, "pk: 17 bits of LDS offset, 6 bits per window axis");
+#pragma unroll
+  for (int j = 0; j < ImgRegs<K, TR>::PER; ++j) {
+    const int idx = threadIdx.x + 256 * j;
+    const int c = idx / (ROWS * COLS);
+    const int rem = idx - c * (ROWS * COLS);
+    const int row = rem / COLS, xl = rem - row * COLS;
+    const int dst = (c * 2 + (xl & 1)) * PPV + row * XPV + (xl >> 1);
+    r.pk[j] = idx < TOT ? ((dst << 14) | (c << 12) | (row << 6) | xl) : ((PPV - 1) << 14);
+    if constexpr (VOFF) r.voff[j] = idx < TOT ? (unsigned)((c * H + row) * W + xl) * (unsigned)sizeof(PT) : IMG_DROP;
+  }
+}
+
+template <int K, int PAD, typename PT, bool VOFF, int TR = 16>
+__device__ __forceinline__ void image_request_buf(ImgRegs<K, TR>& r, const PT* __restrict__ img, long long elems, int n, int C, int cg,
+                                                  int H, int W, int oy0, int ox0, bool valid) {
+  constexpr int ROWS = Geo<K, TR>::ROWS, COLS = Geo<K, TR>::COLS, PER = ImgRegs<K, TR>::PER;
+  constexpr bool U8 = sizeof(PT) == 1;
+  const int iy0 = 2 * oy0 - PAD, ix0 = 2 * ox0 - PAD;
+  const long long org = valid ? ((long long)(n * C + cg * 3) * H + iy0) * W + ix0 : 0;
+  const __amdgpu_buffer_rsrc_t rs = raw_buffer(img + org, valid ? (unsigned)((elems - org) * (long long)sizeof(PT)) : 0u);
+  [[maybe_unused]] const int HW4 = H * W * (int)sizeof(PT), W4 = W * (int)sizeof(PT);
+  auto fetch = [&](int j, unsigned off) {
+    if constexpr (U8) r.v[j] = __uint_as_float((unsigned)__builtin_amdgcn_raw_buffer_load_b8(rs, off, 0, 0));
+    else r.v[j] = __uint_as_float(__builtin_amdgcn_raw_buffer_load_b32(rs, off, 0, 0));
+  };
+  auto offset_of = [&](int j, int pk) -> unsigned {
+    if constexpr (VOFF) return r.voff[j];
+    else return mad_u24((unsigned)(pk >> 6) & 63u, W4, mad_u24((unsigned)(pk >> 12) & 3u, HW4, ((unsigned)pk & 63u) * (unsigned)sizeof(PT)));
+  };
+  r.inside = ~0u;
+  if (iy0 >= 0 && ix0 >= 0 && iy0 + ROWS <= H && ix0 + COLS <= W) {
+#pragma unroll
+    for (int j = 0; j < PER; ++j) {
+      int pk = r.pk[j];
+      if constexpr (!VOFF) asm volatile("" : "+v"(pk));
+      fetch(j, offset_of(j, pk));
+    }
+  } else {
+    const int ylo = iy0 < 0 ? -iy0 : 0, xlo = ix0 < 0 ? -ix0 : 0;
+    const unsigned ycnt = (unsigned)((H - iy0 < ROWS ? H - iy0 : ROWS) - ylo), xcnt = (unsigned)((W - ix0 < COLS ? W - ix0 : COLS) - xlo);
+    if constexpr (U8) r.inside = 0;
+#pragma unroll
+    for (int j = 0; j < PER; ++j) {
+      int pk = r.pk[j];
+      asm volatile("" : "+v"(pk));
+      const bool ok = (unsigned)(((pk >> 6) & 63) - ylo) < ycnt && (unsigned)((pk & 63) - xlo) < xcnt;
+      fetch(j, ok ? offset_of(j, pk) : IMG_DROP);
+      if constexpr (U8) r.inside |= (ok ? 1u : 0u) << j;
+    }
+  }
+}
+
+template <int K, bool U8, int TR = 16>
+__device__ __forceinline__ void image_land_buf(float* __restrict__ T, const ImgRegs<K, TR>& r, const float* __restrict__ lut = nullptr) {
+  float val[ImgRegs<K, TR>::PER];
+#pragma unroll
+  for (int j = 0; j < ImgRegs<K, TR>::PER; ++j) {
+    if constexpr (U8) {
+      int pk = r.pk[j];
+      asm volatile("" : "+v"(pk));
+      val[j] = lut[((pk >> 12) & 3) * 256 + (int)__float_as_uint(r.v[j])];
+    } else {
+      val[j] = r.v[j];
+    }
+  }
+#pragma unroll
+  for (int j = 0; j < ImgRegs<K, TR>::PER; ++j) {
+    int dst = r.pk[j];
+    asm volatile("" : "+v"(dst));
+    dst = (int)((unsigned)dst >> 14);
+    if constexpr (U8) T[dst] = ((r.inside >> j) & 1u) ? val[j] : 0.f;
+    else T[dst] = val[j];
+  }
+}
+
+template <int K, int PAD, typename PT, bool BUF>
+__device__ __forceinline__ void conv_request(ImgRegs<K>& nx, const PT* __restrict__ img, long long elems, int n, int C, int cg, int H,
+                                             int W, int oy0, int ox0, bool valid) {
+  if constexpr (BUF) image_request_buf<K, PAD, PT, true>(nx, img, elems, n, C, cg, H, W, oy0, ox0, valid);
+  else image_request<K, PAD, false>(nx, img, n, C, cg, H, W, oy0, ox0, valid);
+}
+template <int K, bool HOIST, bool U8, bool BUF>
+__device__ __forceinline__ void conv_land(float* __restrict__ T, const ImgRegs<K>& nx, const float* __restrict__ lut) {
+  if constexpr (BUF) image_land_buf<K, U8>(T, nx, lut);
+  else image_land<K, HOIST, 16, U8>(T, nx, 1.f, lut);
+}
+
+template <int K, int PAD, bool BNBWD = false, bool MULTI = false, typename PTAG = float>
+__global__ __launch_bounds__(256, 2) void skinny_conv_kernel(const typename Pixel<PTAG>::type* __restrict__ img,
                                                             const float* __restrict__ w_ref,
                                                             float* __restrict__ feat,
                                                             float* __restrict__ stats_partial, int N, int C, int H,
@@ -129,7 +228,10 @@
                                                             const float* __restrict__ y_raw,
                                                             const float* __restrict__ y_bnp, int npg,
                                                             const float* __restrict__ lut = nullptr) {
+  using PT = typename Pixel<PTAG>::type;
+  constexpr bool BUF = Pixel<PTAG>::buf;
   constexpr bool U8 = sizeof(PT) == 1;
+  static_assert(!BUF || (K == 7 && !BNBWD && !MULTI), "buffer staging: conv1 forward with one channel group");
   constexpr int KT = Geo<K>::KT, KS = Geo<K>::KS;
   extern __shared__ __attribute__((aligned(16))) unsigned char smem[];
   float* T = (float*)smem;
@@ -147,8 +249,9 @@
 
   const int tid = threadIdx.x, lane = tid & 63, wave = tid >> 6;
   const int h = lane >> 5, l31 = lane & 31;
-  const int ncg = C / 3;
+  const int ncg = BUF ? 1 : C / 3;
   const int ntiles = N * tiles_y * tiles_x;
+  [[maybe_unused]] const long long img_elems = (long long)N * C * H * W;
 
   auto stage_weights = [&](int cg) {
     for (int idx = tid; idx < KS * 128; idx += 256) {
@@ -167,13 +270,14 @@
   const float* wl0 = Wl + h * 64 + l31;
 
   ImgRegs<K> nx;
-  image_index<K>(nx);
+  if constexpr (BUF) image_index_buf<K, PT, true>(nx, H, W);
+  else image_index<K>(nx);
   if (PIPE && (int)blockIdx.x < ntiles) {
     const int t0 = vtile(blockIdx.x, ntiles);
     const int n = t0 / (tiles_y * tiles_x);
     const int trem = t0 - n * (tiles_y * tiles_x);
-    image_request<K, PAD, false>(nx, img, n, C, 0, H, W, (trem / tiles_x) * 16, (trem % tiles_x) * 16, true);
-    image_land<K, HOIST, 16, U8>(T, nx, 1.f, lut);
+    conv_request<K, PAD, PT, BUF>(nx, img, img_elems, n, C, 0, H, W, (trem / tiles_x) * 16, (trem % tiles_x) * 16, true);
+    conv_land<K, HOIST, U8, BUF>(T, nx, lut);
     if (MULTI) stage_weights(0);
   }
   for (int v = blockIdx.x; v < ntiles; v += gridDim.x) {
@@ -182,12 +286,14 @@
     const int trem = tile - n * (tiles_y * tiles_x);
     const int oy0 = (trem / tiles_x) * 16, ox0 = (trem % tiles_x) * 16;
     f32x16 acc[2][2];
-#pragma unroll
-    for (int a = 0; a < 2; ++a)
-#pragma unroll
-      for (int b = 0; b < 2; ++b)
-#pragma unroll
-        for (int r = 0; r < 16; ++r) acc[a][b][r] = 0.f;
+    if constexpr (!BUF) {
+#pragma unroll
+      for (int a = 0; a < 2; ++a)
+#pragma unroll
+        for (int b = 0; b < 2; ++b)
+#pragma unroll
+          for (int r = 0; r < 16; ++r) acc[a][b][r] = 0.f;
+    }
     const int eg = lane >> 4, eslot = lane & 15;
     f32x4 yv[BNBWD ? 16 : 1];
 
@@ -199,10 +305,10 @@
         if (cg2 == ncg) { cg2 = 0; tile2 = vtile(v + gridDim.x, ntiles); }
         const int n2 = tile2 / (tiles_y * tiles_x);
         const int trem2 = tile2 - n2 * (tiles_y * tiles_x);
-        image_request<K, PAD, false>(nx, img, n2, C, cg2, H, W, (trem2 / tiles_x) * 16, (trem2 % tiles_x) * 16, tile2 < ntiles);
+        conv_request<K, PAD, PT, BUF>(nx, img, img_elems, n2, C, cg2, H, W, (trem2 / tiles_x) * 16, (trem2 % tiles_x) * 16, tile2 < ntiles);
       } else {
-        image_request<K, PAD, false>(nx, img, n, C, cg, H, W, oy0, ox0, true);
-        image_land<K, HOIST, 16, U8>(T, nx, 1.f, lut);
+        conv_request<K, PAD, PT, BUF>(nx, img, img_elems, n, C, cg, H, W, oy0, ox0, true);
+        conv_land<K, HOIST, U8, BUF>(T, nx, lut);
         if (MULTI) stage_weights(cg);
       }
       if (BNBWD && (!MULTI || cg == 0)) {
@@ -222,6 +328,10 @@
         const int ko = h ? koff<K>(KS + s) : koff<K>(s);
         const float a0 = T[pb0 + ko], a1 = T[pb1 + ko];
         const float b0 = wl0[s * 128], b1 = wl0[s * 128 + 32];
+        if (BUF && s == 0) {
+          const f32x16 zero = {0.f, 0.f, 0.f, 0.f, 0.f, 0.f, 0.f, 0.f, 0.f, 0.f, 0.f, 0.f, 0.f, 0.f, 0.f, 0.f};
+          acc[0][0] = acc[0][1] = acc[1][0] = acc[1][1] = zero;
+        }
         acc[0][0] = __builtin_amdgcn_mfma_f32_32x32x2f32(a0, b0, acc[0][0], 0, 0, 0);
         acc[0][1] = __builtin_amdgcn_mfma_f32_32x32x2f32(a0, b1, acc[0][1], 0, 0, 0);
         acc[1][0] = __builtin_amdgcn_mfma_f32_32x32x2f32(a1, b0, acc[1][0], 0, 0, 0);
@@ -229,7 +339,7 @@
       }
       if (PIPE) {
         __syncthreads();
-        image_land<K, HOIST, 16, U8>(T, nx, 1.f, lut);
+        conv_land<K, HOIST, U8, BUF>(T, nx, lut);
         if (MULTI) stage_weights(cg2);
       }
     }
@@ -245,6 +355,9 @@
 #pragma unroll
       for (int i = 0; i < 16; ++i) asm volatile("" : "+v"(yv[BNBWD ? i : 0]));
     }
+    [[maybe_unused]] const __amdgpu_buffer_rsrc_t feat_rs = raw_buffer(feat + (size_t)n * HF * WF * 64, BUF ? (unsigned)(HF * WF * 256) : 0u);
+    auto flush = [&](auto FULL) __attribute__((always_inline)) {
+    constexpr bool full = decltype(FULL)::value;
 #pragma unroll
     for (int rowq = 0; rowq < 4; ++rowq) {
       const int mt = rowq >> 1, half = rowq & 1;
@@ -259,8 +372,18 @@
 #pragma unroll
       for (int it = 0; it < 4; ++it) {
         const int pl = it * 4 + eg, ox = ox0 + pl;
-        const f32x4 v = *(const f32x4*)(Ew + pl * 64 + eslot * 4);
-        if (oy < HF && ox < WF) {
+        f32x4 v = *(const f32x4*)(Ew + pl * 64 + eslot * 4);
+        if constexpr (BUF) {
+          unsigned off = (unsigned)((oy * WF + ox) * 256 + eslot * 16);
+          if constexpr (!full) {
+            const bool ok = oy < HF && ox < WF;
+            off = ok ? off : IMG_DROP;
+            v = ok ? v : f32x4{0.f, 0.f, 0.f, 0.f};
+          }
+          __builtin_amdgcn_raw_buffer_store_b128(v, feat_rs, off, 0, 0);
+#pragma unroll
+          for (int e = 0; e < 4; ++e) { s1[e] += v[e]; s2[e] = __builtin_fmaf(v[e], v[e], s2[e]); }
+        } else if (oy < HF && ox < WF) {
           *(f32x4*)(feat + ((size_t)(n * HF + oy) * WF + ox) * 64 + eslot * 4) = v;
           if (BNBWD) {
             const f32x4 yy = yv[BNBWD ? rowq * 4 + it : 0];
@@ -274,6 +397,9 @@
         }
       }
     }
+    };
+    if (BUF && oy0 + 16 <= HF && ox0 + 16 <= WF) flush(std::true_type{});
+    else flush(std::false_type{});
     if (stats_partial) {
 #pragma unroll
       for (int e = 0; e < 4; ++e) {
@@ -392,13 +518,15 @@
       3,  16,  24,  40,  46,  65,  81,  95,  98, 100, 105, 112, 119, 120, 122, 126,
     127, 128, 129, 132, 133, 134, 135, 136, 139, 142, 143, 145, 146, 255, 255, 255};
 
-template <int K, int PAD, bool FUSED = false, typename PT = float>
-__global__ __launch_bounds__(256, 2) void skinny_wgrad_kernel(const PT* __restrict__ img,
+template <int K, int PAD, bool FUSED = false, typename PTAG = float>
+__global__ __launch_bounds__(256, 2) void skinny_wgrad_kernel(const typename Pixel<PTAG>::type* __restrict__ img,
                                                              const float* __restrict__ feat,
                                                              float* __restrict__ partial, int N, int C, int H, int W,
                                                              int HF, int WF, int tiles_y, int tiles_x,
                                                              const float* __restrict__ feat_bnp, const PoolFuse pf, int npg,
                                                              const float* __restrict__ lut = nullptr) {
+  using PT = typename Pixel<PTAG>::type;
+  constexpr bool BUF = Pixel<PTAG>::buf;
   constexpr bool U8 = sizeof(PT) == 1;
   constexpr int KT = Geo<K>::KT;
   constexpr int NT = (KT + 31) / 32;
@@ -550,11 +678,17 @@
     }
   };
   ImgRegs<K> ir;
-  image_index<K, 16, WXP, WPP>(ir);
+  static_assert(!BUF || (K == 7 && FUSED), "buffer staging: the fused conv1 weight gradient");
+  if constexpr (BUF) image_index_buf<K, PT, false, 16, WXP, WPP>(ir, H, W);
+  else image_index<K, 16, WXP, WPP>(ir);
+  [[maybe_unused]] const long long img_elems = (long long)N * C * H * W;
   auto i_request = [&](int tile_) {
     const int n_ = tile_ / tpi;
     const int trem_ = tile_ - n_ * tpi;
-    image_request<K, PAD, K == 4>(ir, img, n_, C, cg, H, W, (trem_ / tiles_x) * 16, (trem_ % tiles_x) * 16, tile_ < ntiles);
+    if constexpr (BUF)
+      image_request_buf<K, PAD, PT, false>(ir, img, img_elems, n_, C, cg, H, W, (trem_ / tiles_x) * 16, (trem_ % tiles_x) * 16, tile_ < ntiles);
+    else
+      image_request<K, PAD, K == 4>(ir, img, n_, C, cg, H, W, (trem_ / tiles_x) * 16, (trem_ % tiles_x) * 16, tile_ < ntiles);
   };
   if ((int)blockIdx.x < ntiles) { f_request(vtile(blockIdx.x, ntiles), 0); i_request(vtile(blockIdx.x, ntiles)); }
   for (int v = blockIdx.x; v < ntiles; v += gridDim.x) {
@@ -583,7 +717,10 @@
 #pragma unroll 1
     for (int half = 0; half < NSTAGE; ++half) {
       __syncthreads();
-      if (half == 0) image_land<K, K == 4, 16, U8, WXP, WPP>(T, ir, 1.f, lut);
+      if (half == 0) {
+        if constexpr (BUF) image_land_buf<K, U8>(T, ir, lut);
+        else image_land<K, K == 4, 16, U8, WXP, WPP>(T, ir, 1.f, lut);
+      }
       f_resolve();
       __syncthreads();
       if (half + 1 < NSTAGE) f_request(tile, half + 1);
@@ -710,21 +847,33 @@
   return g > ntiles ? ntiles : g;
 }
 
+static bool buffer_staging_ok(const srlz_skinny_desc* d) {
+  if (d->kind != 0 || d->c != 3) return false;
+  const long long bytes = (long long)d->n * d->c * d->himg * d->wimg * 4, lead = (3LL * d->wimg + 3) * 4;
+  return bytes + lead <= (long long)IMG_DROP && (long long)d->himg * d->wimg * 4 < (1LL << 24) &&
+         (long long)d->hf * d->wf * 256 <= (long long)IMG_DROP;
+}
+
 template <int K, int PAD, typename PT = float>
 static int launch_conv(const PT* img, const float* w, float* feat, float* stats, const srlz_skinny_desc* d, hipStream_t st,
-                       const float* y_raw = nullptr, const float* y_bnp = nullptr, const float* lut = nullptr) {
+                       const float* y_raw = nullptr, const float* y_bnp = nullptr, const float* lut = nullptr, bool generic = false) {
   const int ty = (d->hf + 15) / 16, tx = (d->wf + 15) / 16;
   const int ntiles = d->n * ty * tx;
   const bool multi = d->c > 3;
   const dim3 grid(persistent_grid(ntiles)), block(256);
-#define SRLZ_CONV_LAUNCH(BN, MU, PIPED)                                                                                   \
+#define SRLZ_CONV_LAUNCH_KERNEL(KERNEL, PIPED)                                                                            \
   do {                                                                                                                    \
     const size_t lds = conv_lds<K>(PIPED) + (sizeof(PT) == 1 ? 768 * 4 : 0);                                              \
-    SRLZ_MAX_LDS((skinny_conv_kernel<K, PAD, BN, MU, PT>), lds);                                                          \
-    SRLZ_LAUNCH((skinny_conv_kernel<K, PAD, BN, MU, PT>), grid, block, lds, st, img, w, feat, stats, d->n, d->c,          \
+    SRLZ_MAX_LDS(KERNEL, lds);                                                                                            \
+    SRLZ_LAUNCH(KERNEL, grid, block, lds, st, img, w, feat, stats, d->n, d->c,                                            \
                 d->himg, d->wimg, d->hf, d->wf, ty, tx, y_raw, y_bnp, images_per_group(d), lut);                          \
   } while (0)
+#define SRLZ_CONV_LAUNCH(BN, MU, PIPED) SRLZ_CONV_LAUNCH_KERNEL((skinny_conv_kernel<K, PAD, BN, MU, PT>), PIPED)
   bool launched = false;
+  if constexpr (K == 7) if (!generic && buffer_staging_ok(d)) {
+    SRLZ_CONV_LAUNCH_KERNEL((skinny_conv_kernel<K, PAD, false, false, BufStaged<PT>>), true);
+    launched = true;
+  }
   if constexpr (K == 4 && sizeof(PT) == 4) if (y_raw) {
     if (multi) SRLZ_CONV_LAUNCH(true, true, false); else SRLZ_CONV_LAUNCH(true, false, false);
     launched = true;
@@ -733,6 +882,7 @@
     if (multi) SRLZ_CONV_LAUNCH(false, true, true); else SRLZ_CONV_LAUNCH(false, false, true);
   }
 #undef SRLZ_CONV_LAUNCH
+#undef SRLZ_CONV_LAUNCH_KERNEL
   return 0;
 }
 
@@ -746,7 +896,8 @@
 
 template <int K, int PAD, typename PT = float>
 static int launch_wgrad(const PT* img, const float* feat, float* dw, void* ws, size_t ws_bytes, const srlz_skinny_desc* d,
-                        hipStream_t st, const float* feat_bnp = nullptr, const PoolFuse* pfuse = nullptr, const float* lut = nullptr) {
+                        hipStream_t st, const float* feat_bnp = nullptr, const PoolFuse* pfuse = nullptr, const float* lut = nullptr,
+                        bool generic = false) {
   constexpr int NT = (Geo<K>::KT + 31) / 32;
   const int ty = (d->hf + 15) / 16, tx = (d->wf + 15) / 16;
   const int ntiles = d->n * ty * tx;
@@ -759,8 +910,12 @@
   if (pfuse) pf = *pfuse;
   bool launched = false;
   if constexpr (K == 7) if (pf.y) {
-    SRLZ_LAUNCH((skinny_wgrad_kernel<K, PAD, true, PT>), dim3(g, d->c / 3), dim3(256), lds, st, img, feat, partial, d->n, d->c, d->himg,
-                d->wimg, d->hf, d->wf, ty, tx, feat_bnp, pf, images_per_group(d), lut);
+    if (!generic && buffer_staging_ok(d))
+      SRLZ_LAUNCH((skinny_wgrad_kernel<K, PAD, true, BufStaged<PT>>), dim3(g, d->c / 3), dim3(256), lds, st, img, feat, partial, d->n, d->c,
+                  d->himg, d->wimg, d->hf, d->wf, ty, tx, feat_bnp, pf, images_per_group(d), lut);
+    else
+      SRLZ_LAUNCH((skinny_wgrad_kernel<K, PAD, true, PT>), dim3(g, d->c / 3), dim3(256), lds, st, img, feat, partial, d->n, d->c, d->himg,
+                  d->wimg, d->hf, d->wf, ty, tx, feat_bnp, pf, images_per_group(d), lut);
     launched = true;
   }
   if (!launched)
@@ -784,20 +939,45 @@
   return persistent_grid(d->n * ((d->hf + 15) / 16) * ((d->wf + 15) / 16));
 }
 
-extern "C" int srlz_conv1_fwd(const float* x_nchw, const float* w_ref, float* y_nhwc, float* stats_partial,
-                              const srlz_skinny_desc* d, srlz_stream_t stream) {
+extern "C" int srlz_conv1_buffer_staging_supported(const srlz_skinny_desc* d) {
+  if (check_skinny(d)) return 0;
+  return buffer_staging_ok(d) ? 1 : 0;
+}
+
+static int conv1_fwd(const float* x_nchw, const float* w_ref, float* y_nhwc, float* stats_partial, const srlz_skinny_desc* d,
+                     srlz_stream_t stream, bool generic) {
   if (int rc = check_skinny(d)) return rc;
   SRLZ_REQUIRE(d->kind == 0, SRLZ_ERR_BAD_DESC, "conv1_fwd: descriptor kind must be 0");
   SRLZ_REQUIRE(x_nchw && w_ref && y_nhwc, SRLZ_ERR_NULL, "conv1_fwd: null pointer");
-  return launch_conv<7, 3>(x_nchw, w_ref, y_nhwc, stats_partial, d, as_stream(stream));
-}
-
-extern "C" int srlz_conv1_fwd_u8(const uint8_t* x_u8, const float* norm_lut, const float* w_ref, float* y_nhwc,
-                                 float* stats_partial, const srlz_skinny_desc* d, srlz_stream_t stream) {
+  return launch_conv<7, 3>(x_nchw, w_ref, y_nhwc, stats_partial, d, as_stream(stream), nullptr, nullptr, nullptr, generic);
+}
+
+static int conv1_fwd_u8(const uint8_t* x_u8, const float* norm_lut, const float* w_ref, float* y_nhwc, float* stats_partial,
+                        const srlz_skinny_desc* d, srlz_stream_t stream, bool generic) {
   if (int rc = check_skinny(d)) return rc;
   SRLZ_REQUIRE(d->kind == 0, SRLZ_ERR_BAD_DESC, "conv1_fwd_u8: descriptor kind must be 0");
   SRLZ_REQUIRE(x_u8 && norm_lut && w_ref && y_nhwc, SRLZ_ERR_NULL, "conv1_fwd_u8: null pointer");
-  return launch_conv<7, 3, uint8_t>(x_u8, w_ref, y_nhwc, stats_partial, d, as_stream(stream), nullptr, nullptr, norm_lut);
+  return launch_conv<7, 3, uint8_t>(x_u8, w_ref, y_nhwc, stats_partial, d, as_stream(stream), nullptr, nullptr, norm_lut, generic);
+}
+
+extern "C" int srlz_conv1_fwd(const float* x_nchw, const float* w_ref, float* y_nhwc, float* stats_partial,
+                              const srlz_skinny_desc* d, srlz_stream_t stream) {
+  return conv1_fwd(x_nchw, w_ref, y_nhwc, stats_partial, d, stream, false);
+}
+
+extern "C" int srlz_conv1_fwd_u8(const uint8_t* x_u8, const float* norm_lut, const float* w_ref, float* y_nhwc,
+                                 float* stats_partial, const srlz_skinny_desc* d, srlz_stream_t stream) {
+  return conv1_fwd_u8(x_u8, norm_lut, w_ref, y_nhwc, stats_partial, d, stream, false);
+}
+
+extern "C" int srlz_debug_conv1_fwd_generic(const float* x_nchw, const float* w_ref, float* y_nhwc, float* stats_partial,
+                                            const srlz_skinny_desc* d, srlz_stream_t stream) {
+  return conv1_fwd(x_nchw, w_ref, y_nhwc, stats_partial, d, stream, true);
+}
+
+extern "C" int srlz_debug_conv1_fwd_u8_generic(const uint8_t* x_u8, const float* norm_lut, const float* w_ref, float* y_nhwc,
+                                               float* stats_partial, const srlz_skinny_desc* d, srlz_stream_t stream) {
+  return conv1_fwd_u8(x_u8, norm_lut, w_ref, y_nhwc, stats_partial, d, stream, true);
 }
 
 extern "C" size_t srlz_skinny_bwd_weight_workspace(const srlz_skinny_desc* d) {
@@ -831,7 +1011,7 @@
 static int conv1_bwd_weight_fused(const PT* x_nchw, const float* lut, const float* y_nhwc, const float* bnp, const uint8_t* argmax,
                                   const float* dpooled, const float* sums, int training, float* dw_ref, void* ws,
                                   size_t ws_bytes, const srlz_skinny_desc* d, const srlz_pool_desc* pd,
-                                  srlz_stream_t stream) {
+                                  srlz_stream_t stream, bool generic = false) {
   if (int rc = check_skinny(d)) return rc;
   SRLZ_REQUIRE(d->kind == 0 && pd, SRLZ_ERR_BAD_DESC, "conv1_bwd_weight_fused: descriptor kind must be 0");
   SRLZ_REQUIRE(x_nchw && y_nhwc && bnp && argmax && dpooled && sums && dw_ref && ws, SRLZ_ERR_NULL,
@@ -843,7 +1023,7 @@
   pf.y = y_nhwc; pf.argmax = argmax; pf.dpooled = dpooled; pf.bnp = bnp; pf.sums = sums;
   pf.HP = pd->hp; pf.WP = pd->wp; pf.pad = pd->pool_pad; pf.training = training;
   pf.inv_count = 1.0f / (float)((double)images_per_group(d) * d->hf * d->wf);
-  return launch_wgrad<7, 3, PT>(x_nchw, y_nhwc, dw_ref, ws, ws_bytes, d, as_stream(stream), nullptr, &pf, lut);
+  return launch_wgrad<7, 3, PT>(x_nchw, y_nhwc, dw_ref, ws, ws_bytes, d, as_stream(stream), nullptr, &pf, lut, generic);
 }
 
 extern "C" int srlz_conv1_bwd_weight_fused(const float* x_nchw, const float* y_nhwc, const float* bnp, const uint8_t* argmax,
@@ -861,6 +1041,24 @@
   SRLZ_REQUIRE(norm_lut, SRLZ_ERR_NULL, "conv1_bwd_weight_fused_u8: null normalisation table");
   return conv1_bwd_weight_fused<uint8_t>(x_u8, norm_lut, y_nhwc, bnp, argmax, dpooled, sums, training, dw_ref, ws, ws_bytes, d, pd,
                                          stream);
+}
+
+extern "C" int srlz_debug_conv1_bwd_weight_fused_generic(const float* x_nchw, const float* y_nhwc, const float* bnp,
+                                                         const uint8_t* argmax, const float* dpooled, const float* sums, int training,
+                                                         float* dw_ref, void* ws, size_t ws_bytes, const srlz_skinny_desc* d,
+                                                         const srlz_pool_desc* pd, srlz_stream_t stream) {
+  return conv1_bwd_weight_fused<float>(x_nchw, nullptr, y_nhwc, bnp, argmax, dpooled, sums, training, dw_ref, ws, ws_bytes, d, pd,
+                                       stream, true);
+}
+
+extern "C" int srlz_debug_conv1_bwd_weight_fused_u8_generic(const uint8_t* x_u8, const float* norm_lut, const float* y_nhwc,
+                                                            const float* bnp, const uint8_t* argmax, const float* dpooled,
+                                                            const float* sums, int training, float* dw_ref, void* ws, size_t ws_bytes,
+                                                            const srlz_skinny_desc* d, const srlz_pool_desc* pd,
+                                                            srlz_stream_t stream) {
+  SRLZ_REQUIRE(norm_lut, SRLZ_ERR_NULL, "debug_conv1_bwd_weight_fused_u8_generic: null normalisation table");
+  return conv1_bwd_weight_fused<uint8_t>(x_u8, norm_lut, y_nhwc, bnp, argmax, dpooled, sums, training, dw_ref, ws, ws_bytes, d, pd,
+                                         stream, true);
 }
 
 extern "C" int srlz_convT_out_bwd_data(const float* dy_nchw, const float* w_ref, float* dx_nhwc, const float* x_raw,
diff --git a/srl-zoo_amd/srlz/_cabi.py b/srl-zoo_amd/srlz/_cabi.py
--- a/srl-zoo_amd/srlz/_cabi.py
+++ b/srl-zoo_amd/srlz/_cabi.py
@@ -91,6 +91,11 @@
     "srlz_conv64_bwd_weight_plan": (c_int, [_C64, c_int, c_int, POINTER(c_int)]),
     "srlz_conv64_bwd_fused_workgroups": (c_int, [_C64]),
     "srlz_conv1_workgroups": (c_int, [_SK]),
+    "srlz_conv1_buffer_staging_supported": (c_int, [_SK]),
+    "srlz_debug_conv1_fwd_generic": (c_int, [P, P, P, P, _SK, P]),
+    "srlz_debug_conv1_fwd_u8_generic": (c_int, [P, P, P, P, P, _SK, P]),
+    "srlz_debug_conv1_bwd_weight_fused_generic": (c_int, [P, P, P, P, P, P, c_int, P, P, c_size_t, _SK, _PD, P]),
+    "srlz_debug_conv1_bwd_weight_fused_u8_generic": (c_int, [P, P, P, P, P, P, P, c_int, P, P, c_size_t, _SK, _PD, P]),
     "srlz_convT_out_os_plan": (c_int, [_SK, c_int, POINTER(c_int)]),
     "srlz_conv64_debug_program": (c_int, [_C64, c_int, POINTER(c_int), c_int]),
     "srlz_linear_debug_route": (c_int, [c_int, c_int, c_int, c_int, c_int, P, P, c_int, c_size_t, POINTER(c_int)]),
@@ -247,7 +252,8 @@
                "srlz_conv64_wino_tiles", "srlz_conv64_wino_bwd_data_rows",
                "srlz_conv64_debug_program", "srlz_comm_world", "srlz_dense_supported",
                "srlz_dense_out_fwd_loss_workgroups", "srlz_reward_probe_chunk_rows", "srlz_infer_block_supported",
-               "srlz_infer_tile", "srlz_conv64_bwd_fused_workgroups", "srlz_conv1_workgroups"}
+               "srlz_infer_tile", "srlz_conv64_bwd_fused_workgroups", "srlz_conv1_workgroups",
+               "srlz_conv1_buffer_staging_supported"}
 
 EXPORTED = sorted(_PROTOS.keys())
 
```
